# ComputationalRobotics/XM-code

Measured on AMD Instinct MI355X. Metric: BM iters/sec (tCG Hessian-vector iterations per second; ms_per_step = wall-clock-to-KKT of one staircase solve), higher is better.
Workload: dtype f64

## Files before the change

xm-code_amd/csrc/xm_common.h:

```cpp
#pragma once

#include <hip/hip_runtime.h>

#include <cstdint>
#include <cstdio>
#include <stdexcept>
#include <string>
#include <vector>

namespace xm {

struct Error : std::runtime_error {
    int code;
    Error(int c, const std::string &m) : std::runtime_error(m), code(c) {}
};

#define XM_HIP_CHECK(expr)                                                                            \
    do {                                                                                              \
        hipError_t _e = (expr);                                                                       \
        if (_e != hipSuccess)                                                                         \
            throw ::xm::Error(-3, std::string("HIP error: ") + hipGetErrorString(_e) + " at " +       \
                                      __FILE__ + ":" + std::to_string(__LINE__) + " (" #expr ")");    \
    } while (0)

// ... 76 lines not shown
    double *ksum;
    unsigned int *kcount;
    int nt_cam0;
    int rev;
    struct Cand { const double *R, *s; double *G, *egs, *S0, *rgR, *rgs, *partials; } cand;
};

enum Epilogue { EPI_PLAIN = 0, EPI_GRAD = 1, EPI_HESS = 2, EPI_CERT = 3, EPI_AUTO = 4 };
__host__ __device__ inline CamArgs cand_args(const CamArgs &a) {
    CamArgs b = a;
    b.R = a.cand.R; b.s = a.cand.s; b.G = a.cand.G; b.egs = a.cand.egs; b.S0 = a.cand.S0; b.rgR = a.cand.rgR; b.rgs = a.cand.rgs;
    b.partials = a.cand.partials;
    return b;
}

constexpr int kMaxPeers = 8;
struct PeerXchg {
    int world = 0, rank = 0;
    double *buf[kMaxPeers] = {};
    unsigned long long *flag[kMaxPeers] = {};
    unsigned long long *ticket = nullptr;
    unsigned long long *err = nullptr;
    long long spin_ticks = 0;
    unsigned long long epoch_base = 0;
    int mute = 0;
    int lite = 0;
};

struct PointPtrs { double *G, *egs, *S0, *rgR, *rgs; };
struct OuterStepArgs {
    int nloc, cam0;
    const TcgScal *scal_cur;
    TcgScal *scal_next;
    const OuterScal *os_cur;
    OuterScal *os_next;
    const double *parts;
    double *partsB_out;
    int nA, nB;
    const double *HpR, *Hps;
    double *R, *s;
    double *Rc, *sc;
    double *pR;
    const double *ps_cur;
    double *ps_next;
    double *vR, *vs, *HvR, *Hvs, *rR;
    const double *rs_cur;
    double *rs_next;
    double *Wloc, *Wpad;
    PointPtrs cur, cand;
    const double *partsA;
    double *partsM;
    int nM;
    double delta_bar, gradtol;
    int max_outer;
    double *trace;
    int trace_cap;
    const int *stop_req;
    unsigned long long *hprog;
    unsigned int run;
    int slot, grp;
};
void launch_outer_step(int o, int polar, const OuterStepArgs &A, int grid, hipStream_t st);

void launch_qw_dense(int o, int epi, const double *Q, int64_t ld, const double *W, double alpha, const CamArgs &a,
                     hipStream_t st);
void launch_qw_bsr3(int o, int epi, const int64_t *rowptr, const int32_t *colidx, const double *blocks, const double *W,
                    double alpha, const CamArgs &a, hipStream_t st, int64_t nb = 0, const int4 *rowinfo = nullptr);
int64_t sell_resident_bytes(int64_t stream, int64_t other);
void bsr_build_rowinfo(const int64_t *rowptr_host, int nloc, std::vector<int4> &out);
int qw_grid(int nloc);
void launch_qw_dense_split(int o, int epi, const double *Q, int64_t ld, const double *W, double alpha, const CamArgs &a, hipStream_t st);
int qw_dense_tile_cols();
int qw_dense_split_k(int nloc, int64_t ld);
int bsr_grid(int nloc);
size_t sym_prow_count(int nloc, int64_t ld, int o);
size_t sym_pcol_count(int nloc, int64_t ld, int o);
void qw_bench_nt(int nt);
void symv_bench_k(int k, int kf);
int symv_trace_slots();
void launch_qw_sym_traced(int o, const double *Q, int64_t ld, const double *W, const CamArgs &a, double *Prow, double *Pcol, unsigned long long *trace,
                          int grid[2], hipStream_t st);
void symv_plan_get(int nloc, int64_t ld, int out[4]);
void launch_qw_sym(int o, int epi, const double *Q, int64_t ld, const double *W, double alpha, const CamArgs &a, double *Prow,
                   double *Pcol, hipStream_t st, int rev = 0);
void launch_asym(const double *Q, int64_t ld, int64_t m, double *out, int grid, hipStream_t st);
void launch_dense_to_f32(const double *src, float *dst, int64_t rows, int64_t ld, unsigned int *bad, hipStream_t st);
void launch_qw_dense_f32(int o, int epi, const float *Qf, const double *Qd, int64_t ld, const double *W, double alpha, const CamArgs &a, hipStream_t st);
void launch_qw_sym_f32(int o, int epi, const float *Qf, const double *Qd, int64_t ld, const double *W, double alpha, const CamArgs &a, double *Prow,
                       double *Pcol, hipStream_t st, int rev = 0);

void launch_symhash(const double *Q, int64_t ld, int64_t row0, int64_t nrows, int64_t m, unsigned long long *out, int grid, hipStream_t st);

void launch_transpose_pad(const double *src_colmajor, int64_t lds, int64_t rows, int64_t cols, double *dst, int64_t ldd,
                          hipStream_t st);
void launch_dense_from_bsr(const int64_t *rowptr, const int32_t *colidx, const double *blocks, int64_t nloc, int64_t cam0,
                           double *dst, int64_t ldd, hipStream_t st);

int flat_grid(int64_t elems);
void launch_scale_rows(int o, int nloc, const double *R, const double *s, double *Wloc, hipStream_t st);
void launch_tcg_init(int o, int nloc, const double *rgR, const double *rgs, const double *R, const double *s, double *rR,
                     double *rs, double *pR, double *ps, double *vR, double *vs, double *HvR, double *Hvs, double *Wloc,
                     TcgScal *scal0, double rr, double delta, unsigned long long *hstat, hipStream_t st, double *Wpad = nullptr, int seq = 0,
                     const SpecCtl *spec = nullptr);
void launch_cg_step(int o, int nloc, const TcgScal *scal_cur, TcgScal *scal_next, const double *parts, int nA_loc, int nB_loc, int world,
                    const double *HpR, const double *Hps, const double *R, const double *s, double *pR,
                    const double *ps_cur, double *ps_next, double *vR, double *vs, double *HvR, double *Hvs, double *rR, const double *rs_cur,
                    double *rs_next, double *Wloc, double *partsB_out, unsigned long long *hstat, int b_off, int64_t mat, double *Afull,
                    double *Wfull, int grouping, const struct PeerXchg &xchg, hipStream_t st, double *Wpad = nullptr);
struct OuterArgs { double loss, delta, delta_bar, gradtol; int shrink_count, last_iter; };
void launch_outer_finalize(const double *partsA, int nA_loc, int world, const double *partsM, int nM, const TcgScal *scal, double *hres,
                           unsigned long long seq, int grouping, hipStream_t st, const OuterArgs *oa = nullptr, SpecCtl *spec_out = nullptr);
void launch_retract(int o, int nloc, int cam0, const double *R, const double *s, const double *D, const double *ds, double t,
                    double *Rout, double *sout, double *Wloc, hipStream_t st, int polar = 0);
int retract_grid(int nloc);
void launch_retract_model(int o, int nloc, int cam0, const double *R, const double *s, const double *vR, const double *vs, double *Rout, double *sout,
                          double *Wloc, double *Wpad, const double *HvR, const double *Hvs, const double *rgR, const double *rgs, double *parts,
                          hipStream_t st, int polar);
void launch_cert_prepare(int o, int nloc, int cam0, double lam, const double *QsR, const double *R, const double *s,
                         double *Lam, double *dz, double *parts, hipStream_t st);
void launch_recover_gram(int64_t n, int r, const double *R, const double *s, double *parts, int grid, hipStream_t st);
void launch_recover_project(int64_t n, int r, const double *R, const double *s, const double *V, double *rot, double *scale, int *negcount,
                            hipStream_t st, int variant = 0);
void launch_negate(double *x, int64_t len, hipStream_t st);
int dots_multi_segments(int64_t len);
void launch_dots_multi(const double *V, int64_t ldv, int m, const double *w, int64_t len, double *c, double *scratch, hipStream_t st);
void launch_sub_vc(double *w, const double *V, int64_t ldv, const double *c, int m, int64_t len, hipStream_t st);
void launch_scale_copy(double *dst, const double *src, double a, int64_t len, hipStream_t st);
void launch_copy_words(void *dst, const void *src, size_t bytes, hipStream_t st);
void launch_lz_alpha(const double *c1j, const double *c2j, double *alpha_j, hipStream_t st);
void launch_dots_multi_parts(const double *V, int64_t ldv, int m, const double *w, int64_t len, double *scratch, hipStream_t st);
bool lz_fused_ok(int m);
void launch_sub_vc_fin(double *w, const double *V, int64_t ldv, const double *parts, int m, int64_t len, double *c_out, const double *c_prev,
                       double *alpha_j, hipStream_t st);
void launch_lz_next_fin(double *dst, const double *w, const double *parts, double *beta_j, int64_t len, hipStream_t st);
void launch_lz_next(double *dst, const double *w, const double *ww, double *beta_j, int64_t len, hipStream_t st);
void launch_gemv_n(double *y, const double *V, int64_t ldv, const double *c, int m, int64_t len, hipStream_t st);


void launch_edge_locate(int64_t ne, const int32_t *ei, const int32_t *ej, int cam0, int nloc, const int64_t *rowptr, const int32_t *colidx,
                        int64_t *pos_ij, int64_t *pos_ji, int64_t *pos_d, hipStream_t st);
void launch_edge_write(bool dense, int64_t ne, const int32_t *ei, const int32_t *ej, const double *M, const double *w, int cam0, int nloc,
                       const int64_t *inc_ptr, const int32_t *inc_edge, const int64_t *pos_ij, const int64_t *pos_ji, const int64_t *pos_d,
                       double *blocks, double *Q, int64_t ld, hipStream_t st);
void launch_edge_residual(int64_t ne, const int32_t *ei, const int32_t *ej, const double *M, const double *Y, int o, int OP, double *res,
                          hipStream_t st);

void launch_xm2_error(int64_t n, const double *w, const double *res, double *err, hipStream_t st);
void launch_radix_hist(int64_t n, const double *x, int shift, unsigned long long prefix, unsigned int *hist, hipStream_t st);
void launch_xm2_filter(int64_t n, const double *err, const double *w, double thr, double *wout, unsigned int *removed, hipStream_t st);

#define XM_DISPATCH_O(o, CALL)                                                         \
    switch (o) {                                                                       \
        case 1: { constexpr int O_ = 1; CALL; } break;                                 \
        case 3: { constexpr int O_ = 3; CALL; } break;                                 \
        case 4: { constexpr int O_ = 4; CALL; } break;                                 \
        case 5: { constexpr int O_ = 5; CALL; } break;                                 \
        case 6: { constexpr int O_ = 6; CALL; } break;                                 \
        case 7: { constexpr int O_ = 7; CALL; } break;                                 \
        case 8: { constexpr int O_ = 8; CALL; } break;                                 \
        case 9: { constexpr int O_ = 9; CALL; } break;                                 \
        case 10: { constexpr int O_ = 10; CALL; } break;                               \
        default: throw Error(-2, "rank o must be 1 or 3..10, got " + std::to_string(o)); \
    }

inline void check_launch(const char *what) {
    hipError_t e = hipGetLastError();
    if (e != hipSuccess) throw Error(-3, std::string("kernel launch failed (") + what + "): " + hipGetErrorString(e));
}

}
```

xm-code_amd/csrc/xm_kernels.hip:

```cpp
#include <algorithm>
#include <cmath>
#include <cstdlib>
#include <cstring>
#include <type_traits>

#include "xm_common.h"
#include "xm_device.h"

namespace xm {

__device__ __forceinline__ double2 nt_load16(const double2 *p) {
    typedef double d2v __attribute__((ext_vector_type(2)));
    const d2v v = __builtin_nontemporal_load(reinterpret_cast<const d2v *>(p));
    return make_double2(v.x, v.y);
}

template <int O, int EPI, int NSUB, bool SPLIT = false>
__global__ __launch_bounds__(256) void qw_dense_kernel(const double *__restrict__ Q, int64_t ld,
                                                        const double *__restrict__ W, double alpha, CamArgs a) {
    constexpr int OP = pitch_of(O);
    int role = EPI;
    constexpr int TILE = NSUB * 128;
    constexpr int TILE2 = TILE * OP / 2;
    constexpr int NST = (TILE2 + 255) / 256;
// ... 743 lines not shown
                for (int k = 0; k < O; ++k) acc[r][k] += q[3 * r] * w[0][k] + q[3 * r + 1] * w[1][k] + q[3 * r + 2] * w[2][k];
        }
        if (VAR >= 1) {
            __builtin_amdgcn_fence(__ATOMIC_ACQ_REL, "wavefront");
            __builtin_amdgcn_wave_barrier();
        }
    }
    EpiOps eops;
    BSR_TS(5);
    epi_prefetch<O, EPI>(eops, active ? cam : 0, gl, active, a, (EPI == EPI_AUTO) ? role : (int)EPI);
    qw_finish<O, EPI, 16, kBsrRows>(cam, gl, slot, active, acc, alpha, a, eops, red, (EPI == EPI_AUTO) ? role : (int)EPI);
    BSR_TS(6);
}
#ifdef XM_BSR_TRACE
extern "C" void xm_bsr_trace_set(unsigned long long *p) { (void)hipMemcpyToSymbol(HIP_SYMBOL(g_bsr_trace), &p, sizeof(p)); }
#endif

__global__ __launch_bounds__(256) void transpose_pad_kernel(const double *__restrict__ src, int64_t lds, int64_t rows,
                                                             int64_t cols, double *__restrict__ dst, int64_t ldd) {
    __shared__ double tile[32][33];
    const int tx = threadIdx.x & 31, ty = threadIdx.x >> 5;
    const int64_t r0 = (int64_t)blockIdx.y * 32, c0 = (int64_t)blockIdx.x * 32;
#pragma unroll
    for (int j = 0; j < 32; j += 8) {
        const int64_t r = r0 + tx, c = c0 + ty + j;
        tile[ty + j][tx] = (r < rows && c < cols) ? src[r + c * lds] : 0.0;
    }
    __syncthreads();
#pragma unroll
    for (int j = 0; j < 32; j += 8) {
        const int64_t r = r0 + ty + j, c = c0 + tx;
        if (r < rows && c < ldd) dst[r * ldd + c] = (c < cols) ? tile[tx][ty + j] : 0.0;
    }
}

__global__ void dense_from_bsr_kernel(const int64_t *__restrict__ rowptr, const int32_t *__restrict__ colidx,
                                      const double *__restrict__ blocks, int64_t nloc, int64_t cam0, double *dst, int64_t ldd) {
    const int64_t cam = blockIdx.x;
    if (cam >= nloc) return;
    for (int64_t b = rowptr[cam0 + cam] + threadIdx.x / 9; b < rowptr[cam0 + cam + 1]; b += blockDim.x / 9) {
        const int e = threadIdx.x % 9;
        if (threadIdx.x / 9 < (int)(blockDim.x / 9))
            dst[(cam * 3 + e / 3) * ldd + (int64_t)colidx[b] * 3 + e % 3] = blocks[b * 9 + e];
    }
}

#pragma clang fp contract(off)
__device__ __forceinline__ unsigned long long pack_stat(int seq, int iter, int status) {
    return ((unsigned long long)(unsigned)seq << 32) | ((unsigned long long)((unsigned)iter & 0xffffffu) << 8) | (unsigned long long)(unsigned)(status & 0xff);
}
__device__ __forceinline__ void publish_host(unsigned long long *hstat, unsigned long long v) {
    if (hstat) __hip_atomic_store(hstat, v, __ATOMIC_RELAXED, __HIP_MEMORY_SCOPE_SYSTEM);
}

struct StepDecision {
    int mode;
    double step;
};
__device__ __forceinline__ StepDecision tcg_decide(const TcgScal &sc, double pHp) {
    StepDecision d;
    const double alpha = sc.rr / pHp;
    if (sc.rr < 1e-15) { d.mode = 5; d.step = 0.0; return d; }
    const bool neg = alpha <= 0.0;
    if (neg || sc.vv + 2.0 * alpha * sc.vp + alpha * alpha * sc.pp > sc.delta * sc.delta) {
        const double sq = sqrt(sc.vp * sc.vp + sc.pp * (sc.delta * sc.delta - sc.vv));
        d.mode = neg ? 1 : 2;
        d.step = (-sc.vp + sq) / sc.pp;
        return d;
    }
    d.mode = 0; d.step = alpha;
    return d;
}

template <int O>
__global__ __launch_bounds__(256) void scale_rows_kernel(int nloc, const double *__restrict__ R, const double *__restrict__ s,
                                                          double *__restrict__ Wloc) {
    constexpr int OP = pitch_of(O);
    const int64_t total = (int64_t)nloc * 3 * OP;
    for (int64_t i = (int64_t)blockIdx.x * 256 + threadIdx.x; i < total; i += (int64_t)gridDim.x * 256)
        Wloc[i] = R[i] * s[i / (3 * OP)];
}

template <int O>
__global__ __launch_bounds__(256) void tcg_init_kernel(int nloc, const double *__restrict__ rgR, const double *__restrict__ rgs,
                                                        const double *__restrict__ R, const double *__restrict__ s,
                                                        double *rR, double *rs, double *pR, double *ps, double *vR, double *vs,
                                                        double *HvR, double *Hvs, double *Wloc, TcgScal *scal0, double rr,
                                                        double delta, unsigned long long *hstat, double *Wpad, int seq, const SpecCtl *spec) {
    constexpr int OP = pitch_of(O);
    const int64_t total = (int64_t)nloc * 3 * OP;
    if (spec != nullptr) {
        if (!spec->go) {
            if (blockIdx.x == 0 && threadIdx.x == 0) { TcgScal sc = *scal0; sc.status = 9; sc.seq = seq; *scal0 = sc; }
            return;
        }
        rr = spec->rr; delta = spec->delta;
    }
    for (int64_t i = (int64_t)blockIdx.x * 256 + threadIdx.x; i < total; i += (int64_t)gridDim.x * 256) {
        const int cam = (int)(i / (3 * OP));
        const double g = rgR[i], gs = rgs[cam];
        rR[i] = g; pR[i] = -g; vR[i] = 0.0; HvR[i] = 0.0;
        const double wv = s[cam] * (-g) + (-gs) * R[i];
        if (Wloc) Wloc[i] = wv;
        if (Wpad) Wpad[(size_t)cam * 16 + (i - (int64_t)cam * (3 * OP))] = wv;
        if (i % (3 * OP) == 0) { rs[cam] = gs; ps[cam] = -gs; vs[cam] = 0.0; Hvs[cam] = 0.0; }
    }
    if (blockIdx.x == 0 && threadIdx.x == 0) {
        TcgScal sc = {};
        sc.rr = rr; sc.vv = 0.0; sc.vp = 0.0; sc.pp = rr; sc.delta = delta; sc.gradnorm = sqrt(rr); sc.last_step = 0.0; sc.model = 0.0;
        sc.status = 0; sc.iter = 0; sc.seq = seq;
        *scal0 = sc;
        publish_host(hstat, pack_stat(seq, 0, 0));
    }
}

template <int O>
__global__ __launch_bounds__(256) void cg_step_kernel(int nloc, const TcgScal *__restrict__ scal_cur, TcgScal *scal_next,
                                                       const double *__restrict__ parts, int nA_loc, int nB_loc, int world,
                                                       const double *__restrict__ HpR,
                                                       const double *__restrict__ Hps, const double *__restrict__ R,
                                                       const double *__restrict__ s, double *pR, const double *__restrict__ ps_cur,
                                                       double *ps_next, double *vR, double *vs, double *HvR, double *Hvs, double *rR,
                                                       const double *__restrict__ rs_cur, double *rs_next, double *Wloc,
                                                       double *partsB_out, unsigned long long *hstat, int b_off, int64_t mat,
                                                       double *Afull, double *Wfull, int grp, PeerXchg x, double *Wpad) {
    constexpr int OP = pitch_of(O);
    __shared__ double sh[4];
    __shared__ double sh16[16];
    __shared__ int sh_flag;
    const int64_t total = (int64_t)nloc * 3 * OP;
    const int64_t stride = (int64_t)gridDim.x * 256;
    int64_t i = (int64_t)blockIdx.x * 256 + threadIdx.x;
    const bool in0 = i < total;
    const int camf = (int)(i / (3 * OP));
    const bool own0 = in0 && (i % (3 * OP) == 0);
    double hp = 0, pv = 0, vv0 = 0, hv = 0, rv = 0, Rv = 0, hs = 0, psv = 0, rsv = 0, sv = 1, vsv = 0, hvs = 0;
    const bool keep_hv = HvR != nullptr;
    if (in0) { hp = HpR[i]; pv = pR[i]; vv0 = vR[i]; if (keep_hv) hv = HvR[i]; rv = rR[i]; Rv = R[i]; hs = Hps[camf]; psv = ps_cur[camf]; rsv = rs_cur[camf]; sv = s[camf]; }
    if (own0) { vsv = vs[camf]; if (keep_hv) hvs = Hvs[camf]; }
    const bool can_pre = x.world <= 1;
    PartialsPre pre;
    if (can_pre) sum_partials_prefetch(parts + b_off, parts + b_off + nA_loc, parts + b_off + 2 * nA_loc, nA_loc, parts + b_off + 3 * nA_loc, nB_loc, pre, grp);
    const TcgScal sc0 = *scal_cur;
    const bool lead = (blockIdx.x == 0 && threadIdx.x == 0);
    if (sc0.status != 0) {
        if (lead) *scal_next = sc0;
        return;
    }
    if (x.world > 1) {
        const int par = sc0.iter & 1;
        const size_t chunk_d = (size_t)b_off + 3 * (size_t)nA_loc + nB_loc;
        const size_t off = ((size_t)par * x.world + x.rank) * chunk_d;
        const unsigned long long epoch = x.epoch_base + (unsigned long long)sc0.iter + 1ull;
        const double *src = x.buf[x.rank] + off;
        if (x.lite) {
            for (int p = 0; p < x.world; ++p) {
                if (p == x.rank) continue;
                double *dst = x.buf[p] + off;
                for (size_t j = (size_t)blockIdx.x * 256 + threadIdx.x; j < chunk_d; j += (size_t)stride)
                    __hip_atomic_store(dst + j, src[j], __ATOMIC_RELAXED, __HIP_MEMORY_SCOPE_SYSTEM);
            }
            asm volatile("s_waitcnt vmcnt(0)" ::: "memory");
            __syncthreads();
            if (threadIdx.x == 0) {
                const unsigned long long t = __hip_atomic_fetch_add(x.ticket + par, 1ull, __ATOMIC_RELAXED, __HIP_MEMORY_SCOPE_AGENT);
                sh_flag = (t + 1 == gridDim.x);
                if (sh_flag) __hip_atomic_store(x.ticket + par, 0ull, __ATOMIC_RELAXED, __HIP_MEMORY_SCOPE_AGENT);
            }
            __syncthreads();
            if (sh_flag && !x.mute && threadIdx.x < x.world && (int)threadIdx.x != x.rank)
                __hip_atomic_store(x.flag[threadIdx.x] + par * kMaxPeers + x.rank, epoch, __ATOMIC_RELAXED, __HIP_MEMORY_SCOPE_SYSTEM);
        } else {
            for (int p = 0; p < x.world; ++p) {
                if (p == x.rank) continue;
                double *dst = x.buf[p] + off;
                for (size_t j = (size_t)blockIdx.x * 256 + threadIdx.x; j < chunk_d; j += (size_t)stride) dst[j] = src[j];
            }
            __threadfence_system();
            asm volatile("s_waitcnt vmcnt(0)" ::: "memory");
            __syncthreads();
            if (threadIdx.x == 0) {
                const unsigned long long t = __hip_atomic_fetch_add(x.ticket + par, 1ull, __ATOMIC_ACQ_REL, __HIP_MEMORY_SCOPE_AGENT);
                sh_flag = (t + 1 == gridDim.x);
                if (sh_flag) __hip_atomic_store(x.ticket + par, 0ull, __ATOMIC_RELAXED, __HIP_MEMORY_SCOPE_AGENT);
            }
            __syncthreads();
            if (sh_flag && !x.mute && threadIdx.x < x.world && (int)threadIdx.x != x.rank) {
                __threadfence_system();
                asm volatile("s_waitcnt vmcnt(0)" ::: "memory");
// ... 64 lines not shown
            const double rsn = rsv + step * hs;
            rR[i] = rn;
            acc += rn * rn;
            if (newdir) {
                const double pn = beta * pv - rn;
                const double psn = beta * psv - rsn;
                pR[i] = pn;
                if (!Afull) {
                    const double wv = sv * pn + psn * Rv;
                    if (Wloc) Wloc[i] = wv;
                    if (Wpad) Wpad[(size_t)camf * 16 + (i - (int64_t)camf * (3 * OP))] = wv;
                }
                if (own0) ps_next[camf] = psn;
            }
            if (own0) { rs_next[camf] = rsn; const double q = rsn / sv; acc += q * q; }
        }
        if (own0) { vs[camf] = vsv + step * psv; if (keep_hv) Hvs[camf] = hvs + step * hs; }
    }
    for (i += stride; i < total; i += stride) {
        const int cam = (int)(i / (3 * OP));
        const bool own = (i % (3 * OP) == 0);
        const double hpi = HpR[i], pi = pR[i], hsi = Hps[cam], psi = ps_cur[cam];
        vR[i] += step * pi;
        if (keep_hv) HvR[i] += step * hpi;
        if (cg) {
            const double rn = rR[i] + step * hpi;
            const double rsn = rs_cur[cam] + step * hsi;
            rR[i] = rn;
            acc += rn * rn;
            if (newdir) {
                const double pn = beta * pi - rn;
                const double psn = beta * psi - rsn;
                pR[i] = pn;
                if (!Afull) {
                    const double wv = s[cam] * pn + psn * R[i];
                    if (Wloc) Wloc[i] = wv;
                    if (Wpad) Wpad[(size_t)cam * 16 + (i - (int64_t)cam * (3 * OP))] = wv;
                }
                if (own) ps_next[cam] = psn;
            }
            if (own) { rs_next[cam] = rsn; const double q = rsn / s[cam]; acc += q * q; }
        }
        if (own) { vs[cam] += step * psi; if (keep_hv) Hvs[cam] += step * hsi; }
    }
    if (Afull && newdir) {
        const int64_t full = mat * world;
        const bool first = (sc0.iter == 0);
        for (int64_t j = (int64_t)blockIdx.x * 256 + threadIdx.x; j < full; j += stride) {
            const int64_t r = j / mat;
            const double b = parts[(size_t)r * chunk + (size_t)(j - r * mat)];
            const double w = Wfull[j];
            const double an = (first ? -w : Afull[j]) + step * b;
            Afull[j] = an;
            Wfull[j] = beta * w - an;
        }
    }
    if (cg) {
        const double tot = block_sum256(acc, sh);
        if (threadIdx.x == 0) partsB_out[blockIdx.x] = tot;
    }
    if (lead) {
        TcgScal nx = sc;
        nx.last_step = step;
        if (!keep_hv) nx.model = sc.model - step * sc.rr + 0.5 * step * step * pHp;
        if (!cg) {
            nx.status = d.mode;
        } else {
            nx.rr = rr_est;
            nx.vv = sc.vv + 2.0 * step * sc.vp + step * step * sc.pp;
            nx.vp = beta * (sc.vp + step * sc.pp);
            nx.pp = beta * beta * sc.pp + rr_est;
            if (conv) {
                nx.status = 3;
            } else {
                nx.iter = sc.iter + 1;
                nx.status = (nx.iter >= kMaxInner) ? 6 : 0;
            }
        }
        *scal_next = nx;
        publish_host(hstat, pack_stat(nx.seq, nx.iter, nx.status));
    }
}

__global__ __launch_bounds__(256) void outer_finalize_kernel(const double *__restrict__ partsA, int nA_loc, int world,
                                                              const double *__restrict__ partsM, int nM,
                                                              const TcgScal *__restrict__ scal, double *hres, unsigned long long seq, int grp,
                                                              OuterArgs oa, SpecCtl *spec_out) {
    __shared__ double sh[4];
    double f = 0.0, rr = 0.0;
    for (int r = 0; r < world; ++r) {
        f += sum_partials256(partsA + (size_t)r * 2 * nA_loc, nA_loc, sh, grp);
        rr += sum_partials256(partsA + (size_t)r * 2 * nA_loc + nA_loc, nA_loc, sh, grp);
    }
    const double m_vec = (nM > 0) ? sum_partials256(partsM, nM, sh, grp) : 0.0;
    if (threadIdx.x == 0) {
        const TcgScal sc = *scal;
        const double m = (nM > 0) ? m_vec : sc.model;
        __hip_atomic_store(hres + 0, f, __ATOMIC_RELAXED, __HIP_MEMORY_SCOPE_SYSTEM);
        __hip_atomic_store(hres + 1, rr, __ATOMIC_RELAXED, __HIP_MEMORY_SCOPE_SYSTEM);
        __hip_atomic_store(hres + 2, m, __ATOMIC_RELAXED, __HIP_MEMORY_SCOPE_SYSTEM);
        __hip_atomic_store(hres + 3, (double)sc.status, __ATOMIC_RELAXED, __HIP_MEMORY_SCOPE_SYSTEM);
        __hip_atomic_store(hres + 4, (double)sc.iter, __ATOMIC_RELAXED, __HIP_MEMORY_SCOPE_SYSTEM);
        if (spec_out != nullptr) {
            const int endreason = (sc.status == 0) ? 6 : sc.status;
            double delta = oa.delta;
            int shrink = oa.shrink_count;
            bool go = (m < 0.0) && endreason != 7;
            if (go) {
                const double rou = (f - oa.loss) / m;
                if (rou < 0.25) { delta *= 0.25; shrink++; }
                else if (rou > 0.75 && endreason <= 2) { delta = fmin(delta * 2, oa.delta_bar); shrink = 0; }
                else shrink = 0;
                bool stop_delta = false;
                if (shrink > 3) { delta *= 1e-3; shrink = 0; if (delta < 1e-20) stop_delta = true; }
                const bool reject = (f > oa.loss || rou < 0.1);
                go = !stop_delta && !reject && endreason != 5 && !(sqrt(rr) < oa.gradtol) && !oa.last_iter;
            }
            SpecCtl sp;
            sp.go = go ? 1 : 0; sp.pad_ = 0; sp.rr = rr; sp.delta = delta;
            *spec_out = sp;
            __hip_atomic_store(hres + 6, go ? 1.0 : 0.0, __ATOMIC_RELAXED, __HIP_MEMORY_SCOPE_SYSTEM);
            __hip_atomic_store(hres + 7, delta, __ATOMIC_RELAXED, __HIP_MEMORY_SCOPE_SYSTEM);
        }
        __atomic_thread_fence(__ATOMIC_SEQ_CST);
        asm volatile("s_waitcnt vmcnt(0)" ::: "memory");
        __hip_atomic_store(reinterpret_cast<unsigned long long *>(hres + 5), seq, __ATOMIC_RELEASE, __HIP_MEMORY_SCOPE_SYSTEM);
    }
}

__device__ __forceinline__ double det3(const double (&M)[3][3]);
template <int O>
__device__ __forceinline__ void polar_rows(double (&X)[3][O]) {
    for (int it = 0; it < 40; ++it) {
        double G[3][3];
#pragma unroll
        for (int a = 0; a < 3; ++a)
#pragma unroll
            for (int b = a; b < 3; ++b) {
                double tt = 0.0;
#pragma unroll
                for (int k = 0; k < O; ++k) tt += X[a][k] * X[b][k];
                G[a][b] = tt; G[b][a] = tt;
            }
        const double d = det3(G);
        if (!(d > 0.0)) return;
        double C[3][3];
        C[0][0] = G[1][1] * G[2][2] - G[1][2] * G[2][1]; C[0][1] = G[0][2] * G[2][1] - G[0][1] * G[2][2]; C[0][2] = G[0][1] * G[1][2] - G[0][2] * G[1][1];
        C[1][1] = G[0][0] * G[2][2] - G[0][2] * G[2][0]; C[1][2] = G[0][2] * G[1][0] - G[0][0] * G[1][2]; C[2][2] = G[0][0] * G[1][1] - G[0][1] * G[1][0];
        C[1][0] = C[0][1]; C[2][0] = C[0][2]; C[2][1] = C[1][2];
        double Y[3][O], nx = 0.0, ny = 0.0;
#pragma unroll
        for (int a = 0; a < 3; ++a)
#pragma unroll
            for (int k = 0; k < O; ++k) {
                const double y = (C[a][0] * X[0][k] + C[a][1] * X[1][k] + C[a][2] * X[2][k]) / d;
                Y[a][k] = y; nx += X[a][k] * X[a][k]; ny += y * y;
            }
        const double g = sqrt(sqrt(ny / nx));
        double delta = 0.0;
#pragma unroll
        for (int a = 0; a < 3; ++a)
#pragma unroll
            for (int k = 0; k < O; ++k) {
                const double z = 0.5 * (g * X[a][k] + Y[a][k] / g);
                delta += (z - X[a][k]) * (z - X[a][k]);
                X[a][k] = z;
            }
        if (delta < 1e-31) return;
    }
}

template <int O, int POLAR>
__device__ __forceinline__ void retract_rows(double (&q)[3][O]) {
    if constexpr (POLAR) {
        polar_rows<O>(q);
    } else {
#pragma unroll
        for (int i = 0; i < 3; ++i) {
            double qq = 0.0;
#pragma unroll
            for (int k = 0; k < O; ++k) qq += q[i][k] * q[i][k];
            qq = sqrt(qq);
#pragma unroll
            for (int k = 0; k < O; ++k) q[i][k] /= qq;
#pragma unroll
            for (int j = i + 1; j < 3; ++j) {
                double uu = 0.0;
#pragma unroll
                for (int k = 0; k < O; ++k) uu += q[i][k] * q[j][k];
#pragma unroll
                for (int k = 0; k < O; ++k) q[j][k] -= uu * q[i][k];
            }
        }
    }
}

struct ModelArgs { const double *HvR, *Hvs, *rgR, *rgs; double *parts; };
template <int O, int POLAR, bool MV = false>
__global__ __launch_bounds__(256) void retract_kernel(int nloc, int cam0, const double *__restrict__ R, const double *__restrict__ s,
                                                       const double *__restrict__ D, const double *__restrict__ ds, double t,
                                                       double *Rout, double *sout, double *Wloc, double *Wpad, ModelArgs mv) {
    constexpr int OP = pitch_of(O);
    __shared__ double sh_mv[4];
    const int cam = blockIdx.x * 256 + threadIdx.x;
    const bool live = cam < nloc;
    if constexpr (!MV) {
        if (!live) return;
    }
    const size_t base = (size_t)(live ? cam : 0) * 3 * OP;
    double q[3][O];
// ... 952 lines not shown
    }
}
void launch_qw_dense(int o, int epi, const double *Q, int64_t ld, const double *W, double alpha, const CamArgs &a, hipStream_t st) {
    if (a.nloc <= 0) return;
    if (a.ks > 1 && a.ksum && a.kcount) {
        XM_DISPATCH_O(o, (qw_dense_ks_o<O_>(epi, Q, ld, W, alpha, a, st)));
        check_launch("qw_dense_ks");
        return;
    }
    if (epi == EPI_CERT) {
        if (o != 1) throw Error(-2, "certificate operator needs o == 1");
        CamArgs ac = a;
        ac.nt_cam0 = qw_nt_cam0(a.nloc, ld);
        hipLaunchKernelGGL((qw_dense_kernel<1, EPI_CERT, 2>), dim3(qw_grid(a.nloc)), dim3(256), 0, st, Q, ld, W, alpha, ac);
    } else {
        XM_DISPATCH_O(o, (qw_dense_epi<O_, kQwNsub>(epi, Q, ld, W, alpha, a, st)));
    }
    check_launch("qw_dense");
}

static int64_t symv_live_groups(int64_t nsteps, int64_t nstrips, int64_t k) {
    int64_t live = 0;
    for (int64_t s = 0; s < nstrips; ++s) live += (std::min<int64_t>(nsteps, (s * kSvStrip + kSvStrip + 5) / 6) + 4 * k - 1) / (4 * k);
    return live;
}
int symv_k(int nloc, int64_t ld) {
    const int64_t nsteps = (nloc + 1) / 2, nstrips = (ld + kSvStrip - 1) / kSvStrip;
    int64_t total = 0;
    for (int64_t s = 0; s < nstrips; ++s) total += std::min<int64_t>(nsteps, (s * kSvStrip + kSvStrip + 5) / 6);
    int64_t k = (int64_t)(std::sqrt((double)total) / 18.0 + 0.5);
    k = std::min<int64_t>(64, std::max<int64_t>(2, k));
    if (symv_live_groups(nsteps, nstrips, k) <= 1100) {
        int64_t ks = 4;
        while (symv_live_groups(nsteps, nstrips, ks) > 504) ++ks;
        k = ks;
    }
    return (int)k;
}
size_t sym_prow_count(int nloc, int64_t ld, int o) { return (size_t)((ld + kSvStrip - 1) / kSvStrip) * 6 * (size_t)((nloc + 1) / 2) * o; }
static int g_symv_k = 0, g_symv_kf = 0;
void symv_bench_k(int k, int kf) { g_symv_k = k; g_symv_kf = kf; }
struct SymvPlan { int K, Kf, ysplit, nchunks, gx, gy; };
static SymvPlan symv_plan(int nloc, int64_t ld) {
    SymvPlan p;
    p.K = g_symv_k > 0 ? g_symv_k : symv_k(nloc, ld);
    const int nsteps = (nloc + 1) / 2, nstrips = (int)((ld + kSvStrip - 1) / kSvStrip);
    p.gy = (nstrips + 1) / 2;
    if (g_symv_k > 0 && g_symv_kf > 0) {
        p.Kf = std::min(g_symv_kf, p.K);
        p.ysplit = (int)(0.75 * p.gy);
    } else if (p.K >= 8 && symv_live_groups(nsteps, nstrips, p.K) > 1100) {
        p.Kf = p.K / 4;
        p.ysplit = (int)(0.75 * p.gy);
    } else {
        p.Kf = p.K; p.ysplit = p.gy;
    }
    auto groups = [&](int s, int k) { return (int)((std::min<int64_t>(nsteps, ((int64_t)s * kSvStrip + kSvStrip + 5) / 6) + 4 * k - 1) / (4 * k)); };
    p.gx = 1;
    for (int y = 0; y < p.gy; ++y) {
        const int k = (y >= p.ysplit) ? p.Kf : p.K, sb = nstrips - 1 - y;
        p.gx = std::max(p.gx, groups(y, k) + (sb != y ? groups(sb, k) : 0));
    }
    p.nchunks = (nsteps + 4 * p.Kf - 1) / (4 * p.Kf);
    return p;
}
void symv_plan_get(int nloc, int64_t ld, int out[4]) {
    const SymvPlan p = symv_plan(nloc, ld);
    out[0] = p.K; out[1] = p.Kf; out[2] = p.ysplit; out[3] = p.nchunks;
}
size_t sym_pcol_count(int nloc, int64_t ld, int o) { return (size_t)symv_plan(nloc, ld).nchunks * (size_t)ld * o; }

static int symv_nt_step0(int nloc, int64_t ld) {
    const double m = 3.0 * nloc;
    const double tri = 8.0 * m * (m + 6.0) / 2.0;
    const int64_t res = qw_resident_bytes((size_t)tri);
    const int nsteps = (nloc + 1) / 2;
    if ((double)res >= tri) return nsteps + 1;
    const double disc = m * m - 2.0 * (double)res / 8.0;
    const double r = m - std::sqrt(std::max(0.0, disc));
    return (int)std::min<double>(nsteps + 1, std::max(0.0, r / 6.0));
}
template <int O>
static void qw_symv_epi(int epi, const double *Q, int64_t ld, const double *W, double alpha, const CamArgs &a, double *Prow, double *Pcol,
                        hipStream_t st, int rev, unsigned long long *trace = nullptr) {
    const SymvPlan pl = symv_plan(a.nloc, ld);
    const int nstrips = (int)((ld + kSvStrip - 1) / kSvStrip);
    const TcgScal *sc = (epi == EPI_HESS || epi == EPI_AUTO) ? a.scal : (const TcgScal *)nullptr;
    const int by_phase = (epi == EPI_AUTO) ? 1 : 0;
    const int ys = pl.ysplit, rK = 4 * pl.K, rKf = 4 * pl.Kf, rys = ys;
    const dim3 gs(pl.gx, pl.gy);
    const int nt0 = symv_nt_step0(a.nloc, ld);
    if (trace) {
        if constexpr (O == 3 || O == 4) hipLaunchKernelGGL((qw_symv_kernel<O, true>), gs, dim3(256), 0, st, Q, ld, W, a.nloc, pl.K, pl.Kf, ys, nt0, sc, Prow, Pcol, trace, rev, by_phase);
    } else hipLaunchKernelGGL((qw_symv_kernel<O>), gs, dim3(256), 0, st, Q, ld, W, a.nloc, pl.K, pl.Kf, ys, nt0, sc, Prow, Pcol, trace, rev, by_phase);
    const dim3 g(qw_grid(a.nloc)), b(256);
    switch (epi) {
        case EPI_PLAIN: hipLaunchKernelGGL((symv_reduce_kernel<O, EPI_PLAIN>), g, b, 0, st, Prow, Pcol, ld, nstrips, rK, rKf, rys, alpha, a); break;
        case EPI_GRAD: hipLaunchKernelGGL((symv_reduce_kernel<O, EPI_GRAD>), g, b, 0, st, Prow, Pcol, ld, nstrips, rK, rKf, rys, alpha, a); break;
        case EPI_HESS: hipLaunchKernelGGL((symv_reduce_kernel<O, EPI_HESS>), g, b, 0, st, Prow, Pcol, ld, nstrips, rK, rKf, rys, alpha, a); break;
        case EPI_AUTO:
            if constexpr (O >= 3) { hipLaunchKernelGGL((symv_reduce_kernel<O, EPI_AUTO>), g, b, 0, st, Prow, Pcol, ld, nstrips, rK, rKf, rys, alpha, a); break; }
            throw Error(-2, "bad epilogue");
        case EPI_CERT:
            if constexpr (O == 1) { hipLaunchKernelGGL((symv_reduce_kernel<1, EPI_CERT>), g, b, 0, st, Prow, Pcol, ld, nstrips, rK, rKf, rys, alpha, a); break; }
            throw Error(-2, "certificate operator needs o == 1");
        default: throw Error(-2, "bad epilogue");
    }
}
int symv_trace_slots() { return kSvTraceSlots; }
void launch_qw_sym_traced(int o, const double *Q, int64_t ld, const double *W, const CamArgs &a, double *Prow, double *Pcol, unsigned long long *trace,
                          int grid[2], hipStream_t st) {
    const SymvPlan pl = symv_plan(a.nloc, ld);
    grid[0] = pl.gx; grid[1] = pl.gy;
    if (trace == nullptr) return;
    if (o == 3) qw_symv_epi<3>(EPI_PLAIN, Q, ld, W, 1.0, a, Prow, Pcol, st, 0, trace);
    else if (o == 4) qw_symv_epi<4>(EPI_PLAIN, Q, ld, W, 1.0, a, Prow, Pcol, st, 0, trace);
    else throw Error(-2, "traced symmetric product: o = 3 or 4");
    check_launch("qw_symv traced");
}

void launch_qw_sym(int o, int epi, const double *Q, int64_t ld, const double *W, double alpha, const CamArgs &a, double *Prow,
                   double *Pcol, hipStream_t st, int rev) {
    if (a.nloc <= 0) return;
    switch (o) {
        case 1: qw_symv_epi<1>(epi, Q, ld, W, alpha, a, Prow, Pcol, st, rev & 1); break;
        case 3: qw_symv_epi<3>(epi, Q, ld, W, alpha, a, Prow, Pcol, st, rev & 1); break;
        case 4: qw_symv_epi<4>(epi, Q, ld, W, alpha, a, Prow, Pcol, st, rev & 1); break;
        case 5: qw_symv_epi<5>(epi, Q, ld, W, alpha, a, Prow, Pcol, st, rev & 1); break;
        default: throw Error(-2, "symmetric product is instantiated for o = 1, 3..5");
    }
    check_launch("qw_symv");
}
__global__ __launch_bounds__(256) void symhash_kernel(const double *__restrict__ Q, int64_t ld, int64_t row0, int64_t nrows, int64_t m,
                                                       unsigned long long *out) {
    __shared__ unsigned long long sh[2][4];
    unsigned long long acc = 0ull, bad = 0ull;
    const int64_t total = nrows * m;
    for (int64_t e = (int64_t)blockIdx.x * 256 + threadIdx.x; e < total; e += (int64_t)gridDim.x * 256) {
        const int64_t lr = e / m, c = e - lr * m, r = row0 + lr;
        if (r >= m || r == c) continue;
        const double v = Q[lr * ld + c];
        if (v != v) bad = 1ull;
        unsigned long long b = (v == 0.0) ? 0ull : (unsigned long long)__double_as_longlong(v);
        unsigned long long z = (unsigned long long)((r < c) ? r : c) * 0x9E3779B97F4A7C15ull + (unsigned long long)((r < c) ? c : r);
        z = (z ^ (z >> 30)) * 0xBF58476D1CE4E5B9ull; z = (z ^ (z >> 27)) * 0x94D049BB133111EBull; z ^= z >> 31;
        const unsigned long long t = (z | 1ull) * b;
        acc += (r < c) ? t : (0ull - t);
    }
    for (int off = 32; off > 0; off >>= 1) { acc += __shfl_xor(acc, off, 64); bad |= __shfl_xor(bad, off, 64); }
    if ((threadIdx.x & 63) == 0) { sh[0][threadIdx.x >> 6] = acc; sh[1][threadIdx.x >> 6] = bad; }
    __syncthreads();
    if (threadIdx.x == 0) {
        out[2 * blockIdx.x] = sh[0][0] + sh[0][1] + sh[0][2] + sh[0][3];
        out[2 * blockIdx.x + 1] = sh[1][0] | sh[1][1] | sh[1][2] | sh[1][3];
    }
}
void launch_symhash(const double *Q, int64_t ld, int64_t row0, int64_t nrows, int64_t m, unsigned long long *out, int grid, hipStream_t st) {
    hipLaunchKernelGGL(symhash_kernel, dim3(grid), dim3(256), 0, st, Q, ld, row0, nrows, m, out);
    check_launch("symhash");
}
void launch_asym(const double *Q, int64_t ld, int64_t m, double *out, int grid, hipStream_t st) {
    hipLaunchKernelGGL(asym_kernel, dim3(grid), dim3(256), 0, st, Q, ld, m, out);
    check_launch("asym");
}

template <int O, int VAR>
static void qw_bsr3_epi(int epi, const int64_t *rp, const int32_t *ci, const double *bl, const double *W, const int4 *ri, double alpha,
                        const CamArgs &a, hipStream_t st) {
    const dim3 g((a.nloc + kBsrRows - 1) / kBsrRows), b(256);
    switch (epi) {
        case EPI_PLAIN: hipLaunchKernelGGL((qw_bsr3_kernel<O, EPI_PLAIN, VAR>), g, b, 0, st, rp, ci, bl, W, ri, alpha, a); break;
        case EPI_GRAD: hipLaunchKernelGGL((qw_bsr3_kernel<O, EPI_GRAD, VAR>), g, b, 0, st, rp, ci, bl, W, ri, alpha, a); break;
        case EPI_HESS: hipLaunchKernelGGL((qw_bsr3_kernel<O, EPI_HESS, VAR>), g, b, 0, st, rp, ci, bl, W, ri, alpha, a); break;
        case EPI_AUTO:
            if constexpr (O >= 3) { hipLaunchKernelGGL((qw_bsr3_kernel<O, EPI_AUTO, VAR>), g, b, 0, st, rp, ci, bl, W, ri, alpha, a); break; }
            throw Error(-2, "bad epilogue");
        default: throw Error(-2, "bad epilogue");
    }
}
static int bsr_nt_cam0(int nloc, int64_t nb) {
    const size_t bytes = (size_t)std::max<int64_t>(nb, 0) * 76;
    return qw_resident_bytes(bytes) >= (int64_t)bytes ? nloc : 0;
}
void bsr_build_rowinfo(const int64_t *rowptr_host, int nloc, std::vector<int4> &out) {
    out.resize((size_t)std::max(nloc, 0));
    for (int c0 = 0; c0 < nloc; c0 += kBsrRows) {
        const int m = std::min(kBsrRows, nloc - c0);
        int order[kBsrRows];
        for (int j = 0; j < m; ++j) order[j] = c0 + j;
        std::stable_sort(order, order + m, [&](int x, int y) {
            return (rowptr_host[x + 1] - rowptr_host[x] + 15) / 16 > (rowptr_host[y + 1] - rowptr_host[y] + 15) / 16;
        });
        for (int j = 0; j < m; ++j) {
            const int i = order[j];
            const int64_t b0 = rowptr_host[i], len = rowptr_host[i + 1] - b0;
            if (len >= ((int64_t)1 << 31)) throw Error(-2, "block-CSR row with 2^31 or more blocks");
            out[(size_t)c0 + j] = make_int4((int)(unsigned)(b0 & 0xffffffffll), (int)(unsigned)((unsigned long long)b0 >> 32), (int)len, i);
        }
    }
}
void launch_qw_bsr3(int o, int epi, const int64_t *rp, const int32_t *ci, const double *bl, const double *W, double alpha,
                    const CamArgs &a0, hipStream_t st, int64_t nb, const int4 *ri) {
    if (a0.nloc <= 0) return;
    CamArgs a = a0;
    a.nt_cam0 = bsr_nt_cam0(a.nloc, nb);
    if (epi == EPI_CERT) {
        if (o != 1) throw Error(-2, "certificate operator needs o == 1");
        hipLaunchKernelGGL((qw_bsr3_kernel<1, EPI_CERT, 0>), dim3((a.nloc + kBsrRows - 1) / kBsrRows), dim3(256), 0, st, rp, ci, bl, W, ri, alpha, a);
    } else {
        switch (o) {
            case 3: qw_bsr3_epi<3, 2>(epi, rp, ci, bl, W, ri, alpha, a, st); break;
            case 4: qw_bsr3_epi<4, 2>(epi, rp, ci, bl, W, ri, alpha, a, st); break;
            case 5: qw_bsr3_epi<5, 2>(epi, rp, ci, bl, W, ri, alpha, a, st); break;
            case 6: qw_bsr3_epi<6, 2>(epi, rp, ci, bl, W, ri, alpha, a, st); break;
            case 1: qw_bsr3_epi<1, 1>(epi, rp, ci, bl, W, ri, alpha, a, st); break;
            case 7: qw_bsr3_epi<7, 1>(epi, rp, ci, bl, W, ri, alpha, a, st); break;
            case 8: qw_bsr3_epi<8, 1>(epi, rp, ci, bl, W, ri, alpha, a, st); break;
            case 9: qw_bsr3_epi<9, 1>(epi, rp, ci, bl, W, ri, alpha, a, st); break;
            case 10: qw_bsr3_epi<10, 1>(epi, rp, ci, bl, W, ri, alpha, a, st); break;
            default: throw Error(-2, "rank o must be 1 or 3..10, got " + std::to_string(o));
        }
    }
    check_launch("qw_bsr3");
}

void launch_transpose_pad(const double *src, int64_t lds, int64_t rows, int64_t cols, double *dst, int64_t ldd, hipStream_t st) {
    const dim3 g((unsigned)((ldd + 31) / 32), (unsigned)((rows + 31) / 32));
    hipLaunchKernelGGL(transpose_pad_kernel, g, dim3(256), 0, st, src, lds, rows, cols, dst, ldd);
    check_launch("transpose_pad");
}
void launch_dense_from_bsr(const int64_t *rp, const int32_t *ci, const double *bl, int64_t nloc, int64_t cam0, double *dst,
                           int64_t ldd, hipStream_t st) {
    hipLaunchKernelGGL(dense_from_bsr_kernel, dim3((unsigned)nloc), dim3(252), 0, st, rp, ci, bl, nloc, cam0, dst, ldd);
    check_launch("dense_from_bsr");
}

void launch_scale_rows(int o, int nloc, const double *R, const double *s, double *Wloc, hipStream_t st) {
    XM_DISPATCH_O(o, hipLaunchKernelGGL((scale_rows_kernel<O_>), dim3(flat_grid((int64_t)nloc * 3 * pitch_of(O_))), dim3(256), 0, st,
                                        nloc, R, s, Wloc));
    check_launch("scale_rows");
}
void launch_tcg_init(int o, int nloc, const double *rgR, const double *rgs, const double *R, const double *s, double *rR, double *rs,
                     double *pR, double *ps, double *vR, double *vs, double *HvR, double *Hvs, double *Wloc, TcgScal *scal0,
                     double rr, double delta, unsigned long long *hstat, hipStream_t st, double *Wpad, int seq, const SpecCtl *spec) {
    XM_DISPATCH_O(o, hipLaunchKernelGGL((tcg_init_kernel<O_>), dim3(flat_grid((int64_t)nloc * 3 * pitch_of(O_))), dim3(256), 0, st,
                                        nloc, rgR, rgs, R, s, rR, rs, pR, ps, vR, vs, HvR, Hvs, Wloc, scal0, rr, delta, hstat, Wpad, seq, spec));
    check_launch("tcg_init");
}
void launch_cg_step(int o, int nloc, const TcgScal *scal_cur, TcgScal *scal_next, const double *parts, int nA_loc, int nB_loc, int world,
                    const double *HpR, const double *Hps, const double *R, const double *s, double *pR,
                    const double *ps_cur, double *ps_next, double *vR, double *vs, double *HvR, double *Hvs, double *rR, const double *rs_cur,
                    double *rs_next, double *Wloc, double *partsB_out, unsigned long long *hstat, int b_off, int64_t mat, double *Afull,
                    double *Wfull, int grouping, const PeerXchg &xchg, hipStream_t st, double *Wpad) {
    XM_DISPATCH_O(o, hipLaunchKernelGGL((cg_step_kernel<O_>), dim3(nB_loc), dim3(256), 0, st, nloc,
                                        scal_cur, scal_next, parts, nA_loc, nB_loc, world, HpR, Hps, R, s, pR, ps_cur, ps_next, vR,
                                        vs, HvR, Hvs, rR, rs_cur, rs_next, Wloc, partsB_out, hstat, b_off, mat, Afull, Wfull, grouping, xchg, Wpad));
    check_launch("cg_step");
}
void launch_outer_finalize(const double *partsA, int nA_loc, int world, const double *partsM, int nM, const TcgScal *scal, double *hres,
                           unsigned long long seq, int grouping, hipStream_t st, const OuterArgs *oa, SpecCtl *spec_out) {
    OuterArgs z;
    std::memset(&z, 0, sizeof(z));
    hipLaunchKernelGGL(outer_finalize_kernel, dim3(1), dim3(256), 0, st, partsA, nA_loc, world, partsM, nM, scal, hres, seq, grouping, oa ? *oa : z,
                       (oa != nullptr) ? spec_out : (SpecCtl *)nullptr);
    check_launch("outer_finalize");
}
void launch_outer_step(int o, int polar, const OuterStepArgs &A, int grid, hipStream_t st) {
    switch (o) {
#define XM_OS_CASE(OO) case OO: if (polar) hipLaunchKernelGGL((outer_step_kernel<OO, 1>), dim3(grid), dim3(256), 0, st, A); \
                                else hipLaunchKernelGGL((outer_step_kernel<OO, 0>), dim3(grid), dim3(256), 0, st, A); break;
        XM_OS_CASE(3) XM_OS_CASE(4) XM_OS_CASE(5) XM_OS_CASE(6) XM_OS_CASE(7) XM_OS_CASE(8) XM_OS_CASE(9) XM_OS_CASE(10)
#undef XM_OS_CASE
        default: throw Error(-2, "device-driven outer iteration: rank o must be 3..10, got " + std::to_string(o));
    }
    check_launch("outer_step");
}
int retract_grid(int nloc) { return (nloc + 255) / 256; }
void launch_retract_model(int o, int nloc, int cam0, const double *R, const double *s, const double *vR, const double *vs, double *Rout, double *sout,
                          double *Wloc, double *Wpad, const double *HvR, const double *Hvs, const double *rgR, const double *rgs, double *parts,
                          hipStream_t st, int polar) {
    const ModelArgs mv = {HvR, Hvs, rgR, rgs, parts};
    const dim3 g(retract_grid(nloc)), b(256);
    if (HvR == nullptr) {
        if (polar) { XM_DISPATCH_O(o, hipLaunchKernelGGL((retract_kernel<O_, 1, false>), g, b, 0, st, nloc, cam0, R, s, vR, vs, 1.0, Rout, sout, Wloc, Wpad, mv)); }
        else { XM_DISPATCH_O(o, hipLaunchKernelGGL((retract_kernel<O_, 0, false>), g, b, 0, st, nloc, cam0, R, s, vR, vs, 1.0, Rout, sout, Wloc, Wpad, mv)); }
        check_launch("retract");
        return;
    }
    if (polar) { XM_DISPATCH_O(o, hipLaunchKernelGGL((retract_kernel<O_, 1, true>), g, b, 0, st, nloc, cam0, R, s, vR, vs, 1.0, Rout, sout, Wloc, Wpad, mv)); }
    else { XM_DISPATCH_O(o, hipLaunchKernelGGL((retract_kernel<O_, 0, true>), g, b, 0, st, nloc, cam0, R, s, vR, vs, 1.0, Rout, sout, Wloc, Wpad, mv)); }
    check_launch("retract_model");
}
void launch_retract(int o, int nloc, int cam0, const double *R, const double *s, const double *D, const double *ds, double t,
                    double *Rout, double *sout, double *Wloc, hipStream_t st, int polar) {
    const ModelArgs mv = {nullptr, nullptr, nullptr, nullptr, nullptr};
    if (polar == 2) {
        XM_DISPATCH_O(o, hipLaunchKernelGGL((retract_quad_kernel<O_>), dim3((nloc + 63) / 64), dim3(256), 0, st, nloc, cam0, R, s, D, ds, t,
                                            Rout, sout, Wloc));
    } else if (polar) {
        XM_DISPATCH_O(o, hipLaunchKernelGGL((retract_kernel<O_, 1>), dim3((nloc + 255) / 256), dim3(256), 0, st, nloc, cam0, R, s, D, ds, t,
                                            Rout, sout, Wloc, (double *)nullptr, mv));
    } else {
        XM_DISPATCH_O(o, hipLaunchKernelGGL((retract_kernel<O_, 0>), dim3((nloc + 255) / 256), dim3(256), 0, st, nloc, cam0, R, s, D, ds, t,
                                            Rout, sout, Wloc, (double *)nullptr, mv));
    }
    check_launch("retract");
}
void launch_cert_prepare(int o, int nloc, int cam0, double lam, const double *QsR, const double *R, const double *s, double *Lam,
                         double *dz, double *parts, hipStream_t st) {
    XM_DISPATCH_O(o, hipLaunchKernelGGL((cert_prepare_kernel<O_>), dim3((nloc + 255) / 256), dim3(256), 0, st, nloc, cam0, lam, QsR, R,
                                        s, Lam, dz, parts));
    check_launch("cert_prepare");
}
void launch_recover_gram(int64_t n, int r, const double *R, const double *s, double *parts, int grid, hipStream_t st) {
    hipLaunchKernelGGL(recover_gram_kernel, dim3(grid), dim3(256), 0, st, n, r, R, s, parts);
    check_launch("recover_gram");
}
void launch_recover_project(int64_t n, int r, const double *R, const double *s, const double *V, double *rot, double *scale, int *negcount,
                            hipStream_t st, int variant) {
    if (variant == 1) hipLaunchKernelGGL(recover_project_wave_kernel, dim3((unsigned)((n + 3) / 4)), dim3(256), 0, st, n, r, R, s, V, rot, scale, negcount);
    else hipLaunchKernelGGL(recover_project_kernel, dim3((unsigned)((n + 255) / 256)), dim3(256), 0, st, n, r, R, s, V, rot, scale, negcount);
    check_launch("recover_project");
}
void launch_negate(double *x, int64_t len, hipStream_t st) {
    hipLaunchKernelGGL(negate_kernel, dim3(flat_grid(len)), dim3(256), 0, st, x, len);
    check_launch("negate");
}
int dots_multi_segments(int64_t len) { return (int)std::min<int64_t>(64, std::max<int64_t>(1, len / 4096)); }
void launch_dots_multi(const double *V, int64_t ldv, int m, const double *w, int64_t len, double *c, double *scratch, hipStream_t st) {
    if (m <= 0) return;
    const int nseg = dots_multi_segments(len);
    if (nseg <= 1 || !scratch) {
        hipLaunchKernelGGL(dots_multi_kernel, dim3(m), dim3(256), 0, st, V, ldv, w, len, c);
    } else {
        const int64_t seg = ((len + nseg - 1) / nseg + 255) / 256 * 256;
        hipLaunchKernelGGL(dots_multi_seg_kernel, dim3(m, nseg), dim3(256), 0, st, V, ldv, w, len, seg, scratch);
        hipLaunchKernelGGL(dots_multi_fin_kernel, dim3((m + 255) / 256), dim3(256), 0, st, scratch, m, nseg, c);
    }
    check_launch("dots_multi");
}
void launch_dots_multi_parts(const double *V, int64_t ldv, int m, const double *w, int64_t len, double *scratch, hipStream_t st) {
    if (m <= 0) return;
    const int nseg = dots_multi_segments(len);
    const int64_t seg = ((len + nseg - 1) / nseg + 255) / 256 * 256;
    hipLaunchKernelGGL(dots_multi_seg_kernel, dim3(m, nseg), dim3(256), 0, st, V, ldv, w, len, seg, scratch);
    check_launch("dots_multi_parts");
}
bool lz_fused_ok(int m) { return m <= kLzMaxCols; }
// ... 354 lines not shown
                run(at(i), qA, wA);
                load_q(at(i + 2), qA, wA);
                run(at(i + 1), qB, wB);
                i += 2;
            }
            if (i + 1 < cnt) {
                load_q(at(i + 1), qB, wB);
                run(at(i), qA, wA);
                run(at(i + 1), qB, wB);
            } else {
                run(at(i), qA, wA);
            }
        }
        return true;
    };
    bool alive;
    const bool nt = jb >= nt_step0;
    if constexpr (AUTO) {
        const int ph = scal->phase;
        if (ph >= PH_STOP) return;
        if (ph == PH_CAND) alive = nt ? sweep(Qd, std::true_type{}) : sweep(Qd, std::false_type{});
        else alive = nt ? sweep(Qf, std::true_type{}) : sweep(Qf, std::false_type{});
    } else {
        alive = nt ? sweep(Qf, std::true_type{}) : sweep(Qf, std::false_type{});
    }
    if (!alive) return;
#pragma unroll
    for (int h = 0; h < 2; ++h)
#pragma unroll
        for (int e = 0; e < 2; ++e)
#pragma unroll
            for (int k = 0; k < O; ++k) L[((h * 2 + e) * O + k) * 64 + lane] = ca[h][e][k];
    __syncthreads();
    if (wave < 2 && lane_ok) {
        double *pc = Pcol + ((size_t)sc * (size_t)ld + (size_t)(cA + 2 * wave)) * O;
#pragma unroll
        for (int e = 0; e < 2; ++e)
#pragma unroll
            for (int k = 0; k < O; ++k) {
                const int idx = ((wave * 2 + e) * O + k) * 64 + lane;
                pc[e * O + k] = ((lds[0][idx] + lds[1][idx]) + lds[2][idx]) + lds[3][idx];
            }
    }
}

void launch_dense_to_f32(const double *src, float *dst, int64_t rows, int64_t ld, unsigned int *bad, hipStream_t st) {
    if (ld % 4 != 0) throw Error(-2, "fp32 copy: leading dimension must be a multiple of 4");
    const size_t n4 = (size_t)rows * (size_t)ld / 4;
    XM_HIP_CHECK(hipMemsetAsync(bad, 0, sizeof(unsigned int), st));
    if (n4 == 0) return;
    const int grid = (int)std::min<size_t>(4096, (n4 + 255) / 256);
    hipLaunchKernelGGL(dense_to_f32_kernel, dim3(grid), dim3(256), 0, st, src, dst, n4, bad);
    check_launch("dense_to_f32");
}

template <int O>
static void qw_dense_f32_epi(int epi, const float *Qf, const double *Qd, int64_t ld, const double *W, double alpha, const CamArgs &a0, hipStream_t st) {
    const dim3 g(qw_grid(a0.nloc)), b(256);
    CamArgs a = a0;
    {
        const size_t row3 = (size_t)3 * (size_t)ld * sizeof(float);
        a.nt_cam0 = (int)std::min<int64_t>(a.nloc, qw_resident_bytes((size_t)a.nloc * row3) / (int64_t)row3);
    }
    switch (epi) {
        case EPI_PLAIN: hipLaunchKernelGGL((qw_dense_f32_kernel<O, EPI_PLAIN>), g, b, 0, st, Qf, Qd, ld, W, alpha, a); break;
        case EPI_HESS: hipLaunchKernelGGL((qw_dense_f32_kernel<O, EPI_HESS>), g, b, 0, st, Qf, Qd, ld, W, alpha, a); break;
        case EPI_AUTO:
            if constexpr (O >= 3) {
                if (!Qd) throw Error(-2, "fp32 product in the device-driven role needs the f64 matrix too");
                hipLaunchKernelGGL((qw_dense_f32_kernel<O, EPI_AUTO>), g, b, 0, st, Qf, Qd, ld, W, alpha, a);
                break;
            }
            throw Error(-2, "bad epilogue");
        default: throw Error(-2, "fp32 dense product: plain, Hessian or device-driven epilogue only");
    }
}
void launch_qw_dense_f32(int o, int epi, const float *Qf, const double *Qd, int64_t ld, const double *W, double alpha, const CamArgs &a, hipStream_t st) {
    if (a.nloc <= 0) return;
    XM_DISPATCH_O(o, (qw_dense_f32_epi<O_>(epi, Qf, Qd, ld, W, alpha, a, st)));
    check_launch("qw_dense_f32");
}
template <int O>
static void qw_symv_f32_epi(int epi, const float *Qf, const double *Qd, int64_t ld, const double *W, double alpha, const CamArgs &a, double *Prow,
                            double *Pcol, hipStream_t st, int rev) {
    const SymvPlan pl = symv_plan(a.nloc, ld);
    const int nstrips = (int)((ld + kSvStrip - 1) / kSvStrip);
    const int rK = 4 * pl.K, rKf = 4 * pl.Kf, ys = pl.ysplit;
    const dim3 gs(pl.gx, pl.gy), g(qw_grid(a.nloc)), b(256);
    int nt0;
    {
        const double m = 3.0 * a.nloc, tri = 4.0 * m * (m + 6.0) / 2.0;
        const int64_t res = qw_resident_bytes((size_t)tri);
        const int nsteps = (a.nloc + 1) / 2;
        if ((double)res >= tri) nt0 = nsteps + 1;
        else {
            const double r = m - std::sqrt(std::max(0.0, m * m - 2.0 * (double)res / 4.0));
            nt0 = (int)std::min<double>(nsteps + 1, std::max(0.0, r / 6.0));
        }
    }
    switch (epi) {
        case EPI_PLAIN:
            hipLaunchKernelGGL((qw_symv_f32_kernel<O, false>), gs, b, 0, st, Qf, Qd, ld, W, a.nloc, pl.K, pl.Kf, ys, nt0, (const TcgScal *)nullptr, Prow, Pcol, rev);
            hipLaunchKernelGGL((symv_reduce_kernel<O, EPI_PLAIN>), g, b, 0, st, Prow, Pcol, ld, nstrips, rK, rKf, ys, alpha, a);
            break;
        case EPI_HESS:
            hipLaunchKernelGGL((qw_symv_f32_kernel<O, false>), gs, b, 0, st, Qf, Qd, ld, W, a.nloc, pl.K, pl.Kf, ys, nt0, a.scal, Prow, Pcol, rev);
            hipLaunchKernelGGL((symv_reduce_kernel<O, EPI_HESS>), g, b, 0, st, Prow, Pcol, ld, nstrips, rK, rKf, ys, alpha, a);
            break;
        case EPI_AUTO:
            if constexpr (O >= 3) {
                if (!Qd) throw Error(-2, "fp32 product in the device-driven role needs the f64 matrix too");
                const int nt64 = symv_nt_step0(a.nloc, ld);
                hipLaunchKernelGGL((qw_symv_f32_kernel<O, true>), gs, b, 0, st, Qf, Qd, ld, W, a.nloc, pl.K, pl.Kf, ys, std::min(nt0, nt64), a.scal, Prow, Pcol, rev);
                hipLaunchKernelGGL((symv_reduce_kernel<O, EPI_AUTO>), g, b, 0, st, Prow, Pcol, ld, nstrips, rK, rKf, ys, alpha, a);
                break;
            }
            throw Error(-2, "bad epilogue");
        default: throw Error(-2, "fp32 symmetric product: plain, Hessian or device-driven epilogue only");
    }
}
void launch_qw_sym_f32(int o, int epi, const float *Qf, const double *Qd, int64_t ld, const double *W, double alpha, const CamArgs &a, double *Prow,
                       double *Pcol, hipStream_t st, int rev) {
    if (a.nloc <= 0) return;
    switch (o) {
        case 3: qw_symv_f32_epi<3>(epi, Qf, Qd, ld, W, alpha, a, Prow, Pcol, st, rev & 1); break;
        case 4: qw_symv_f32_epi<4>(epi, Qf, Qd, ld, W, alpha, a, Prow, Pcol, st, rev & 1); break;
        case 5: qw_symv_f32_epi<5>(epi, Qf, Qd, ld, W, alpha, a, Prow, Pcol, st, rev & 1); break;
        default: throw Error(-2, "fp32 symmetric product is instantiated for o = 3..5");
    }
    check_launch("qw_symv_f32");
}

}
```

xm-code_amd/csrc/xm_sell.h:

```cpp
#pragma once

#include <cstdint>
#include <vector>

#include "xm_solver.h"

namespace xm {

struct SellHost {
    int64_t nloc = 0, ncols = 0;
    int S = 1, lmax = 0;
    bool slice_order = true;
    int64_t nvrows = 0, nslices = 0, nsteps = 0, nparts = 0, nstore = 0;
    std::vector<int64_t> slice_off;
    std::vector<int32_t> slab_start;
    std::vector<uint8_t> kind;
    std::vector<int64_t> src;
    std::vector<int32_t> pslot;
    std::vector<int32_t> ridx;
    std::vector<int64_t> pptr;
    int64_t lines_native72 = 0, lines_native120 = 0, lines_padded = 0;
    std::vector<int64_t> diag_src;
};

void sell_build_host(const int64_t *rowptr, const int32_t *colidx, int64_t nloc, int64_t ncols, int S, int lmax, SellHost &out,
                     int64_t diag_row0 = -1);

enum { SELL_CODEC_FULL = 0, SELL_CODEC_QUAT = 1 };
constexpr int64_t kSellMinBlocks = 2200000;

struct SellArgs {
    const int64_t *slice_off;
    const int32_t *slab_start;
    const int32_t *cols;
    const double *blk;
    const double *diag;
    int64_t row0;
    const int32_t *pslot;
    const int64_t *pptr;
    const int32_t *ridx;
    int S;
    int wstride;
    int coalesced_store;
    int64_t nt_off;
};

class SellMatrix {
public:
    int64_t ncols() const { return ncols_; }
    bool padded_pays(int o) const { return o >= 3 && 3 * pitch_of(o) <= 16 && lines_padded_ * 11 < (3 * pitch_of(o) <= 9 ? lines72_ : lines120_) * 10; }
    SellMatrix(const int64_t *rowptr, const int32_t *colidx, const double *blocks, int64_t nloc, int64_t ncols, int S, int lmax,
               hipStream_t st, int codec = SELL_CODEC_FULL, int64_t row0 = 0);
    int codec() const { return codec_; }
    int64_t stream_bytes() const;
    int64_t nt_off(int o, int64_t nloc) const;
    SellArgs args() const;
    void refill(const int32_t *d_colidx, const double *d_blocks, hipStream_t st);
    double *parts(int o);
    int wstride(int o) const;
    int reduce_gw(int o) const;
    int reduce_grid(int o, int nloc) const;
    int grid() const { return grid_; }
    int64_t nloc() const { return nloc_; }
    int64_t nparts() const { return nparts_; }
    int64_t nsteps() const { return nsteps_; }
    int S() const { return S_; }

private:
    int64_t nloc_ = 0, nparts_ = 0, nsteps_ = 0, nslices_ = 0;
    int S_ = 1, grid_ = 0;
    int64_t ncols_ = 0, max_list_ = 0;
    int64_t lines72_ = 0, lines120_ = 0, lines_padded_ = 0;
    bool coalesced_ = false;
    DevBuf<int64_t> slice_off_, pptr_;
    DevBuf<int32_t> slab_start_, cols_, pslot_, ridx_;
    DevBuf<double> blk_, parts_;
    DevBuf<int64_t> src_;
    DevBuf<uint8_t> kind_;
    int64_t b0_ = 0;
    int parts_o_ = 0;
    int codec_ = SELL_CODEC_FULL;
    int64_t row0_ = 0;
    DevBuf<double> diag_;
    DevBuf<int64_t> diag_src_;
};

void check_viewgraph_blocks(const int64_t *rowptr, const int32_t *colidx, const double *blocks, int64_t nloc, int64_t row0);
void launch_qw_sell(int o, int epi, SellMatrix &m, const double *W, double alpha, const CamArgs &a, int gm, hipStream_t st,
                    const double *Wpad16 = nullptr);
bool sell_supports(int o);
void sell_quat_roundtrip(const double block[9], double quat[4], double rebuilt[9]);

}
```

xm-code_amd/csrc/xm_sell.hip:

```cpp
#include "xm_sell.h"

#include <algorithm>
#include <cstdlib>
#include <cstring>
#include <numeric>
#include <type_traits>

#include "xm_device.h"
#include "xm_sell_codec.h"

namespace xm {

void sell_build_host(const int64_t *rowptr, const int32_t *colidx, int64_t nloc, int64_t ncols, int S, int lmax, SellHost &out,
                     int64_t diag_row0) {
    if (!(S == 1 || S == 2 || S == 4 || S == 8)) throw Error(XM_ERR_ARG, "SELL: slabs must be 1, 2, 4 or 8");
    if (lmax < 2) throw Error(XM_ERR_ARG, "SELL: lmax must be >= 2");
    if (nloc < 0 || ncols < 1 || !rowptr) throw Error(XM_ERR_ARG, "SELL: bad sizes");
    out = SellHost();
    out.nloc = nloc; out.ncols = ncols; out.S = S; out.lmax = lmax;
    const int64_t b0 = rowptr[0], nb = rowptr[nloc] - b0;
    if (nb < 0) throw Error(XM_ERR_ARG, "BSR3: rowptr is not monotone");
    if (nb > 0 && !colidx) throw Error(XM_ERR_ARG, "BSR3: colidx missing");
    std::vector<int64_t> order;
    order.reserve((size_t)nb);
// ... 516 lines not shown
}
template <int GM>
__global__ __launch_bounds__(256) __attribute__((amdgpu_waves_per_eu(4, 4))) void qw_sell_kernel_q_occ4(SellArgs m, const double *__restrict__ W,
                                                                                                      const TcgScal *__restrict__ scal,
                                                                                                      double *__restrict__ parts) {
    qw_sell_entry<3, GM, 0, SELL_CODEC_QUAT>(m, W, scal, parts);
}

int SellMatrix::reduce_gw(int o) const { return (o <= 4 && max_list_ <= 32) ? 4 : 16; }
int SellMatrix::reduce_grid(int o, int nloc) const { const int per = 256 / reduce_gw(o); return (nloc + per - 1) / per; }

template <int O, int EPI, int GW>
__global__ __launch_bounds__(256) void sell_reduce_kernel(const int64_t *__restrict__ pptr, const int32_t *__restrict__ ridx, const double *__restrict__ parts,
                                                           double alpha, CamArgs a, const double *__restrict__ diag, const double *__restrict__ W,
                                                           int64_t row0, int wstride) {
    constexpr int NSLOT = 256 / GW;
    __shared__ double red[NSLOT][3];
    const int gl = threadIdx.x & (GW - 1), slot = threadIdx.x / GW;
    const int cam = blockIdx.x * NSLOT + slot;
    const bool active = cam < a.nloc;
    EpiOps eops;
    epi_prefetch<O, EPI>(eops, active ? cam : 0, gl, active, a);
    const int64_t p0 = active ? pptr[cam] : 0, p1 = active ? pptr[cam + 1] : 0;
    if (EPI == EPI_HESS) {
        if (a.scal->status != 0) return;
    }
    double acc[3][O];
#pragma unroll
    for (int r = 0; r < 3; ++r)
#pragma unroll
        for (int k = 0; k < O; ++k) acc[r][k] = 0.0;
    if (active) {
        for (int64_t p = p0 + gl; p < p1; p += GW) {
            const double *v = parts + (size_t)ridx[p] * 3 * O;
#pragma unroll
            for (int r = 0; r < 3; ++r)
#pragma unroll
                for (int k = 0; k < O; ++k) acc[r][k] += v[r * O + k];
        }
        if (diag != nullptr && !(EPI == EPI_HESS && a.Bout == nullptr) && gl == GW - 1) {
            constexpr int OPW = pitch_of(O);
            const double d = diag[cam];
            const double *w = W + (size_t)(row0 + cam) * wstride;
#pragma unroll
            for (int r = 0; r < 3; ++r)
#pragma unroll
                for (int k = 0; k < O; ++k) acc[r][k] = fma(d, w[r * OPW + k], acc[r][k]);
        }
    }
    if constexpr (EPI == EPI_HESS) {
        if (diag != nullptr && a.Bout == nullptr) {
            Col3 h;
            h.v[0] = h.v[1] = h.v[2] = 0.0;
#pragma unroll
            for (int r = 0; r < 3; ++r)
#pragma unroll
                for (int k = 0; k < O; ++k) {
                    const double t = group_sum<GW>(acc[r][k]);
                    if (gl == k) h.v[r] = t;
                }
            if (active && gl < O) {
                const double d = diag[cam];
#pragma unroll
                for (int r = 0; r < 3; ++r) h.v[r] = alpha * fma(d, eops.s * eops.P.v[r] + eops.ps * eops.R.v[r], h.v[r]);
            }
            qw_tail<O, EPI, GW, NSLOT>(cam, gl, slot, active, h, a, eops, red);
            return;
        }
    }
    qw_finish<O, EPI, GW, NSLOT>(cam, gl, slot, active, acc, alpha, a, eops, red);
}

bool sell_supports(int o) { return o == 1 || (o >= 3 && o <= 5); }
void sell_quat_roundtrip(const double block[9], double quat[4], double rebuilt[9]) {
    double b[9], q[4], r[9];
    for (int e = 0; e < 9; ++e) b[e] = block[e];
    block_to_quat(b, q);
    quat_to_block(q[0], q[1], q[2], q[3], r);
    for (int e = 0; e < 4; ++e) quat[e] = q[e];
    for (int e = 0; e < 9; ++e) rebuilt[e] = r[e];
}

template <int O>
static void qw_sell_o(int epi, SellMatrix &m, const double *W, double alpha, const CamArgs &a, int gm, hipStream_t st, const double *Wpad16) {
    const TcgScal *sc = (epi == EPI_HESS) ? a.scal : (const TcgScal *)nullptr;
    double *parts = m.parts(O);
    SellArgs sa = m.args();
    sa.wstride = m.wstride(O);
    const bool quat = m.codec() == SELL_CODEC_QUAT;
    const bool padded = Wpad16 != nullptr && O >= 3 && 3 * pitch_of(O) <= 16;
    const double *Wn = W;
    const int wn = sa.wstride;
    if (padded) { sa.wstride = 16; W = Wpad16; }
    if (m.grid() > 0) {
        const dim3 g(m.grid()), b(256);
        if (gm != 0 && (uint64_t)m.ncols() * (uint64_t)sa.wstride * 8u >= (1ull << 32)) gm = 0;
        sa.nt_off = m.nt_off(O, a.nloc);
        if (quat) {
            if constexpr (O == 3) {
                if (gm == 1) hipLaunchKernelGGL((qw_sell_kernel_q_occ4<1>), g, b, 0, st, sa, W, sc, parts);
                else hipLaunchKernelGGL((qw_sell_kernel_q_occ4<0>), g, b, 0, st, sa, W, sc, parts);
            } else {
                if (gm == 1) hipLaunchKernelGGL((qw_sell_kernel<O, 1, 0, SELL_CODEC_QUAT>), g, b, 0, st, sa, W, sc, parts);
                else hipLaunchKernelGGL((qw_sell_kernel<O, 0, 0, SELL_CODEC_QUAT>), g, b, 0, st, sa, W, sc, parts);
            }
        } else {
            constexpr int PIPE = (O == 3) ? 1 : 0;
            if (gm == 1) hipLaunchKernelGGL((qw_sell_kernel<O, 1, PIPE>), g, b, 0, st, sa, W, sc, parts);
            else hipLaunchKernelGGL((qw_sell_kernel<O, 0, PIPE>), g, b, 0, st, sa, W, sc, parts);
        }
    }
    const dim3 g(m.reduce_grid(O, a.nloc)), b(256);
#define XM_SELL_REDUCE(GW_)                                                                                                                          \
    switch (epi) {                                                                                                                                  \
        case EPI_PLAIN: hipLaunchKernelGGL((sell_reduce_kernel<O, EPI_PLAIN, GW_>), g, b, 0, st, sa.pptr, sa.ridx, parts, alpha, a, sa.diag, Wn, sa.row0, wn); break; \
        case EPI_GRAD: hipLaunchKernelGGL((sell_reduce_kernel<O, EPI_GRAD, GW_>), g, b, 0, st, sa.pptr, sa.ridx, parts, alpha, a, sa.diag, Wn, sa.row0, wn); break;   \
        case EPI_HESS: hipLaunchKernelGGL((sell_reduce_kernel<O, EPI_HESS, GW_>), g, b, 0, st, sa.pptr, sa.ridx, parts, alpha, a, sa.diag, Wn, sa.row0, wn); break;   \
        default: throw Error(XM_ERR_ARG, "bad epilogue");                                                                                           \
    }
    if (m.reduce_gw(O) == 4) { XM_SELL_REDUCE(4) } else { XM_SELL_REDUCE(16) }
#undef XM_SELL_REDUCE
}

void launch_qw_sell(int o, int epi, SellMatrix &m, const double *W, double alpha, const CamArgs &a, int gm, hipStream_t st, const double *Wpad16) {
    if (a.nloc <= 0) return;
    if (epi == EPI_CERT) {
        if (o != 1) throw Error(XM_ERR_ARG, "certificate operator needs o == 1");
        double *parts = m.parts(1);
        SellArgs sa = m.args();
        sa.wstride = 3;
        if (m.grid() > 0) {
            sa.nt_off = m.nt_off(1, a.nloc);
            if (m.codec() == SELL_CODEC_QUAT) hipLaunchKernelGGL((qw_sell_kernel<1, 0, 0, SELL_CODEC_QUAT>), dim3(m.grid()), dim3(256), 0, st, sa, W, (const TcgScal *)nullptr, parts);
            else hipLaunchKernelGGL((qw_sell_kernel<1, 0>), dim3(m.grid()), dim3(256), 0, st, sa, W, (const TcgScal *)nullptr, parts);
        }
        if (m.reduce_gw(1) == 4) hipLaunchKernelGGL((sell_reduce_kernel<1, EPI_CERT, 4>), dim3(m.reduce_grid(1, a.nloc)), dim3(256), 0, st, sa.pptr, sa.ridx, parts, alpha, a, sa.diag, W, sa.row0, sa.wstride);
        else hipLaunchKernelGGL((sell_reduce_kernel<1, EPI_CERT, 16>), dim3(m.reduce_grid(1, a.nloc)), dim3(256), 0, st, sa.pptr, sa.ridx, parts, alpha, a, sa.diag, W, sa.row0, sa.wstride);
    } else {
        switch (o) {
            case 1: qw_sell_o<1>(epi, m, W, alpha, a, 0, st, nullptr); break;
            case 3: qw_sell_o<3>(epi, m, W, alpha, a, gm, st, Wpad16); break;
            case 4: qw_sell_o<4>(epi, m, W, alpha, a, gm, st, Wpad16); break;
            case 5: qw_sell_o<5>(epi, m, W, alpha, a, gm, st, Wpad16); break;
            default: throw Error(XM_ERR_ARG, "SELL product is instantiated for o = 1, 3, 4, 5");
        }
    }
    check_launch("qw_sell");
}

}
```

xm-code_amd/csrc/xm_solver.h:

```cpp
#pragma once

#include <chrono>
#include <cstdint>
#include <cstdio>
#include <memory>
#include <string>
#include <vector>

#include "../../include/xm_amd.h"
#include "xm_common.h"

namespace xm {

struct Settings {
    int sym = 0;
    int64_t sym_min_rows = 0;
    int64_t sym_rows(int world) const { return sym_min_rows > 0 ? sym_min_rows : (world <= 1 ? 4096 : 6144); }
    int sell = 0;
    int sell_slabs = 4, sell_lmax = 64, sell_gather = 1;
    int sell_codec = 0;
    int sell_wpad = 0;
    int overlap = 0;
    double overlap_min_mb = 64.0;
    int64_t cert_dense_rows = 384;
// ... 146 lines not shown
    int64_t n_landmarks() const;
    void dense_q(double *q, int64_t ldq);
    bool schur_info(int64_t out[3], double *relres) const;
    int schur_precond(int64_t *aggregates, int *block) const;

private:
    int64_t n_ = 0;
    int nloc_ = 0;
    int cam0_ = 0;
    int64_t g0_ = 0;
    int64_t true_loc_ = 0;
    int64_t ntot_ = 0;
    int64_t ld_ = 0;
    int storage_ = XM_STORAGE_DENSE;
    double *dQ_ = nullptr;
    bool ownQ_ = false;
    float *dQ32_ = nullptr;
    void refresh_q32();
    DevBuf<double> Afull_;
    DevBuf<int64_t> rowptr_;
    DevBuf<int32_t> colidx_;
    DevBuf<double> blocks_;
    int64_t nb_loc_ = 0;
    DevBuf<int4> rowinfo_;
    std::unique_ptr<SellMatrix> sell_;
    int sell_gm_ = 0;
    std::unique_ptr<SchurOp> schur_;
    bool schur_dense_ = false;
    int64_t ne_ = 0;
    DevBuf<int32_t> ei_, ej_, inc_edge_;
    DevBuf<int64_t> inc_ptr_, pos_ij_, pos_ji_, pos_d_;
    DevBuf<double> eM_, ew_, eres_;
    bool solved_ = false;
    std::vector<double> w_cur_;
    DevBuf<double> eerr_;
    const double *residuals_recovered_device(const double *rot, const double *scale);
    hipStream_t st_ = nullptr;
    hipStream_t st2_ = nullptr;
    hipEvent_t ev_w_ = nullptr, ev_p_ = nullptr;
    DevBuf<double> Pstrip_;
    bool w_pending_ = false;
    std::shared_ptr<Comm> comm_;
    Settings cfg_;
    PeerXchg xchg_;
    double *partsB_peer_ = nullptr;
    unsigned long long tcg_runs_ = 0;
    std::vector<int64_t> cam_cut_;
    int retraction_ = 0, grouping_ = 0;

    int o_ = 0, OP_ = 0;
    DevBuf<double> R_, s_, Rc_, sc_, W_, D_;
    DevBuf<double> wpad_;
    double *wpad() const { return (wpad_.p && wpad_on_) ? wpad_.p : nullptr; }
    bool wpad_on_ = false;
    const double *wpad_next_ = nullptr;
    PointState ps_[2];
    int cur_ = 0;
    DevBuf<double> rR_, rs_, rsB_, pR_, psA_, psB_, vR_, vs_, HvR_, Hvs_, HpR_, Hps_;
    DevBuf<double> partsA_, partsB_, partsM_;
    DevBuf<double> Prow_, Pcol_;
    DevBuf<double> ksum_;
    DevBuf<unsigned int> kcount_;
    int ks_ = 1;
    std::unique_ptr<SymwProduct> symw_;
    void product_symw(int epi, int o, double alpha, const CamArgs &a);
    bool sym_ok_ = false;
    int sym_max_o_ = 4;
    bool eig_exact_ = false;
    double q_asym_ = 0, q_max_ = 0;
    DevBuf<TcgScal> scal_;
    unsigned long long *hstat_ = nullptr;
    unsigned long long *hstat_dev_ = nullptr;
    double *hpin_ = nullptr;
    double *hpin_dev_ = nullptr;
    size_t hpin_count_ = 0;
    int nA_ = 0, nB_ = 0;
    unsigned long long outer_seq_ = 0;

    const xm_options_t *opt_ = nullptr;
    xm_result_t *res_ = nullptr;
    bool verbose_ = false;
    std::vector<std::pair<hipEvent_t, hipEvent_t>> ev_pool_;
    size_t ev_used_ = 0;
    int64_t hess_launches_ = 0;
    int sym_rev_ = 1;
    std::vector<float> qw_samples_;

    void init(const xm_problem_t &prob);
    void to_host(void *dst, const void *src_dev, size_t bytes);
    void to_dev(void *dst_dev, const void *src, size_t bytes);
    void ensure_pinned(size_t doubles);
    DevBuf<double> lzV_, lzc_, lzw_, lzc2_, lzab_, lzscr_;
    DevBuf<double> recW_;
    int64_t pos_of(int64_t g) const;
    void release_raw();
    void setup_rank(int o);
    void upload_point(const std::vector<double> &R_cm, int o, const std::vector<double> &s_ex);
    void download_point(std::vector<double> &R_cm, std::vector<double> &s_ex);
    CamArgs cam_args(int state) const;
    int prod_grid() const;
    int tcg_blocks() const;
    void product(int epi, int o, double alpha, const CamArgs &a);
    void gather_W();
    void flush_gather();
    bool overlap_applies() const;
    void eval_point(int state, const double *Rp, const double *sp, double &f, double &rr);
    double sum_parts(const double *dparts, int count);
    int run_tcg(double rr, double delta, TcgScal &fin, int adopted = 0);
    int enqueue_spec_tcg();
    void tcg_enqueue_iteration(int i, bool profile);
    bool spec_applies() const;
    DevBuf<SpecCtl> spec_;
    unsigned int tcg_seq_ = 0;
    volatile double *wait_outer_result();
    bool stream_idle(std::chrono::steady_clock::time_point t_wait, const char *what);
    bool agree_any(bool local);
    void drain_events();
    void finish_profile();
    TrResult trust_region(int o, double &gradtol, double linesearch_step, const std::vector<double> &v_dir, double max_time);
    bool device_outer_applies(int o) const;
    TrResult trust_region_device(int o, double &gradtol, double f, double rr, double delta, double delta_bar, double max_time);
    DevBuf<double> trace_dev_;
    DevBuf<int> stop_req_;
    DevBuf<OuterScal> oscal_;
    unsigned int outer_run_ = 0;
    CertResult certificate(int o, double primal, std::vector<double> &v_out);
    int lanczos_min(std::vector<double> &x_out, double &theta, int &iters, double &resid);
    void cert_product(const double *vj, const CamArgs &a, int j);
    void log(const char *fmt, ...) const;
};

class Team {
public:
    Team(const xm_problem_t &prob, int n_gpus, int gpu_map);
    ~Team();
    Team(const Team &) = delete;
    Team &operator=(const Team &) = delete;
    int world() const;
    int comm_kind() const;
    int product_kind(int o) const;
    const std::string &fallback_note() const;
    void solve(const xm_options_t &opt, xm_result_t &res);
    void attach_edges(int64_t ne, const int32_t *ei, const int32_t *ej, const double *M);
    void edge_residuals(double *res);
    void set_edge_weights(const double *w);
    void edge_residuals_recovered(const double *rot, const double *scale, double *res);
    double xm2_filter(const double *rot, const double *scale, double pct, int64_t *removed, double *w_out);
    int64_t cameras() const;
    std::vector<double> weights() const;
private:
    struct Impl;
    std::unique_ptr<Impl> p_;
    void shutdown();
};

}
```

xm-code_amd/csrc/xm_solver.hip:

```cpp
#include "xm_solver.h"
#include "xm_sell.h"
#include "xm_symw.h"
#include "xm_schur.h"
#include "xm_ba.h"
#include "xm_clean.h"

#include <algorithm>
#include <chrono>
#include <cmath>
#include <cstdarg>
#include <cstdlib>
#include <cstring>
#include <thread>

namespace xm {

using clk = std::chrono::steady_clock;
static double secs_since(clk::time_point t0) { return std::chrono::duration<double>(clk::now() - t0).count(); }

void Context::log(const char *fmt, ...) const {
    if (!verbose_ || (comm_ && comm_->rank != 0)) return;
    va_list ap;
    va_start(ap, fmt);
    vprintf(fmt, ap);
// ... 379 lines not shown
            XM_HIP_CHECK(hipMemcpyAsync(repd.p + (size_t)rank * 2, mine2, sizeof(mine2), hipMemcpyHostToDevice, st_));
            comm_->allgather(repd.p, 2, st_);
            std::vector<unsigned long long> all((size_t)world * 2);
            XM_HIP_CHECK(hipMemcpyAsync(all.data(), repd.p, all.size() * sizeof(unsigned long long), hipMemcpyDeviceToHost, st_));
            XM_HIP_CHECK(hipStreamSynchronize(st_));
            unsigned long long tot = 0ull, bad2 = 0ull;
            for (int r = 0; r < world; ++r) { tot += all[(size_t)2 * r]; bad2 |= all[(size_t)2 * r + 1]; }
            if (tot != 0ull || bad2 != 0ull) symw_.reset();
        }
        comm_->host_barrier();
    }
    XM_HIP_CHECK(hipHostMalloc((void **)&hstat_, 256, hipHostMallocMapped | hipHostMallocCoherent));
    std::memset(hstat_, 0, 256);
    XM_HIP_CHECK(hipHostGetDevicePointer((void **)&hstat_dev_, hstat_, 0));
    ensure_pinned((size_t)1 << 17);
    if (viewgraph) {
        attach_edges(prob.ne, prob.edge_i, prob.edge_j, prob.edge_M);
        w_cur_.assign(prob.edge_w, prob.edge_w + prob.ne);
    }
}

Context::~Context() { release_raw(); }

void Context::setup_rank(int o) {
    if (comm_->active()) comm_->host_barrier();
    o_ = o;
    OP_ = pitch_of(o);
    const size_t mat = (size_t)nloc_ * 3 * OP_, vec = (size_t)nloc_;
    const int world = comm_->world;
    const int o_top = std::max(o, (int)std::min<unsigned>(opt_ ? opt_->max_rank : 0u, (unsigned)kMaxRank));
    const size_t mat_top = (size_t)nloc_ * 3 * pitch_of(o_top);
    for (DevBuf<double> *b : {&R_, &Rc_, &D_, &rR_, &pR_, &vR_, &HvR_, &HpR_}) b->ensure(mat, st_, mat_top);
    for (DevBuf<double> *b : {&s_, &sc_, &rs_, &rsB_, &psA_, &psB_, &vs_, &Hvs_, &Hps_}) b->ensure(vec, st_);
    for (int k = 0; k < 2; ++k) {
        ps_[k].G.ensure(mat, st_, mat_top); ps_[k].rgR.ensure(mat, st_, mat_top); ps_[k].egs.ensure(vec, st_); ps_[k].rgs.ensure(vec, st_); ps_[k].S0.ensure(vec * 9, st_);
    }
    cur_ = 0;
    wpad_on_ = sell_ && cfg_.sell_wpad >= 0 && !comm_->active() && sell_supports(o) && o >= 3 && 3 * OP_ <= 16 && (cfg_.sell_wpad == 1 || sell_->padded_pays(o));
    if (wpad_on_ && !wpad_.p) wpad_.alloc((size_t)ntot_ * 16 + 16);
    W_.ensure((size_t)ld_ * OP_ + 16, st_, (size_t)ld_ * pitch_of(o_top) + 16);
    const int nA_loc = prod_grid(), nB_loc = tcg_blocks();
    nA_ = nA_loc * world;
    nB_ = nB_loc * world;
    partsA_.ensure((size_t)3 * nA_, st_);
    const size_t b_off = comm_->active() ? mat : 0;
    const size_t pb = (size_t)2 * (b_off * world + 3 * nA_ + nB_);
    if (comm_->peer() && world > 1 && cfg_.exchange != 1 && !symw_ && storage_ != XM_STORAGE_SCHUR && comm_->device_waits()) {
        partsB_.release();
        comm_->xchg_setup(pb, xchg_);
        partsB_peer_ = xchg_.buf[comm_->rank];
        xchg_.mute = (cfg_.debug_peer_mute && comm_->rank == 1) ? 1 : 0;
        xchg_.lite = cfg_.exchange_lite;
    } else {
        xchg_ = PeerXchg();
        partsB_peer_ = nullptr;
        partsB_.ensure(pb, st_, (size_t)2 * ((comm_->active() ? mat_top : 0) * world + 3 * nA_ + nB_));
    }
    if (comm_->active()) Afull_.ensure(mat * world, st_, mat_top * world); else Afull_.release();
    partsM_.ensure((size_t)std::max(std::max(nB_, flat_grid((int64_t)mat_top) * world), 4 * ((nloc_ + 255) / 256) * world), st_);
    if (sym_ok_ && o >= 3 && o <= sym_max_o_) {
        Prow_.alloc(sym_prow_count(nloc_, ld_, o));
        Pcol_.alloc(sym_pcol_count(nloc_, ld_, o), false);
    } else {
        Prow_.release(); Pcol_.release();
    }
    ks_ = 1;
    if (storage_ == XM_STORAGE_DENSE && !sym_ok_ && cfg_.split_k >= 0) {
        if (cfg_.split_k >= 2) ks_ = std::min(cfg_.split_k, std::max(1, (int)((ld_ + 255) / 256)));
        else if (comm_->active()) ks_ = qw_dense_split_k(nloc_, ld_);
    }
    if (ks_ > 1) {
        ksum_.alloc((size_t)ks_ * mat);
        kcount_.alloc((size_t)qw_grid(nloc_));
    }
    if (overlap_applies()) {
        if (!st2_) {
            XM_HIP_CHECK(hipStreamCreateWithFlags(&st2_, hipStreamNonBlocking));
            XM_HIP_CHECK(hipEventCreateWithFlags(&ev_w_, hipEventDisableTiming));
            XM_HIP_CHECK(hipEventCreateWithFlags(&ev_p_, hipEventDisableTiming));
        }
        Pstrip_.alloc(mat);
    }
    scal_.ensure(2, st_);
    spec_.ensure(1, st_);
    if (sell_ && sell_supports(o)) (void)sell_->parts(o);
    ensure_pinned(std::max<size_t>((size_t)2 * nA_ + (size_t)nB_ + partsM_.count + 64, (size_t)ld_ * OP_ + (size_t)ntot_ + 1024));
    if (comm_->active()) comm_->host_barrier();
}

void Context::upload_point(const std::vector<double> &R_cm, int o, const std::vector<double> &s_ex) {
    const size_t m = (size_t)3 * n_;
    std::vector<double> Rr((size_t)nloc_ * 3 * OP_, 0.0), sl((size_t)nloc_, 1.0);
    for (int c = 0; c < nloc_; ++c) {
        const bool real = c < true_loc_;
        const int64_t g = g0_ + c;
        for (int a = 0; a < 3; ++a)
            for (int k = 0; k < o; ++k)
                Rr[((size_t)c * 3 + a) * OP_ + k] = real ? R_cm[(size_t)(3 * g + a) + (size_t)k * m] : (a == k ? 1.0 : 0.0);
        if (real) sl[(size_t)c] = s_ex[(size_t)g];
    }
    if (cam0_ == 0) sl[0] = 1.0;
    to_dev(R_.p, Rr.data(), Rr.size() * sizeof(double));
    to_dev(s_.p, sl.data(), sl.size() * sizeof(double));
}

void Context::download_point(std::vector<double> &R_cm, std::vector<double> &s_ex) {
    const size_t m = (size_t)3 * n_, mat = (size_t)nloc_ * 3 * OP_;
    std::vector<double> full((size_t)ntot_ * 3 * OP_), sf((size_t)ntot_);
    launch_scale_copy(W_.p + (size_t)comm_->rank * mat, R_.p, 1.0, (int64_t)mat, st_);
    if (comm_->active()) comm_->allgather(W_.p, mat, st_);
    to_host(full.data(), W_.p, full.size() * sizeof(double));
    launch_scale_copy(W_.p + (size_t)comm_->rank * nloc_, s_.p, 1.0, (int64_t)nloc_, st_);
    if (comm_->active()) comm_->allgather(W_.p, (size_t)nloc_, st_);
    to_host(sf.data(), W_.p, sf.size() * sizeof(double));
    XM_HIP_CHECK(hipMemsetAsync(W_.p, 0, W_.count * sizeof(double), st_));
    R_cm.assign(m * (size_t)o_, 0.0);
    s_ex.assign((size_t)n_, 1.0);
    for (int64_t g = 0; g < n_; ++g) {
        const size_t q = (size_t)pos_of(g);
        for (int a = 0; a < 3; ++a)
            for (int k = 0; k < o_; ++k) R_cm[(size_t)(3 * g + a) + (size_t)k * m] = full[(q * 3 + a) * OP_ + k];
        s_ex[(size_t)g] = sf[q];
    }
}

int Context::prod_grid() const {
    if (storage_ == XM_STORAGE_BSR3 && sell_ && sell_supports(o_)) return sell_->reduce_grid(o_, nloc_);
    return (storage_ == XM_STORAGE_BSR3) ? bsr_grid(nloc_) : qw_grid(nloc_);
}

int Context::tcg_blocks() const {
    int g = flat_grid((int64_t)nloc_ * 3 * OP_);
    if (comm_->peer() && comm_->world > 1 && cfg_.exchange != 1 && !symw_ && storage_ != XM_STORAGE_SCHUR && comm_->device_waits()) g = std::min(g, std::max(8, 1024 / std::max(1, comm_->ranks_on_my_device())));
    return g;
}

CamArgs Context::cam_args(int state) const {
    CamArgs a;
    std::memset(&a, 0, sizeof(a));
    a.nloc = nloc_;
    a.cam0 = cam0_;
    a.lam = opt_ ? opt_->lam : 0.0;
    a.R = R_.p;
    a.s = s_.p;
    const PointState &p = ps_[state];
    a.G = p.G.p; a.egs = p.egs.p; a.S0 = p.S0.p; a.rgR = p.rgR.p; a.rgs = p.rgs.p;
    a.pR = pR_.p; a.ps = psA_.p; a.rR = rR_.p; a.rs = rs_.p; a.HpR = HpR_.p; a.Hps = Hps_.p;
    a.Wloc = W_.p + (size_t)cam0_ * 3 * OP_;
    a.out = HpR_.p;
    a.partials = partsA_.p;
    a.scal = scal_.p;
    if (ks_ > 1) { a.ks = ks_; a.ksum = ksum_.p; a.kcount = kcount_.p; }
    return a;
}

void Context::product(int epi, int o, double alpha, const CamArgs &a) {
    if (w_pending_) {
        if (storage_ == XM_STORAGE_DENSE && (epi == EPI_PLAIN || epi == EPI_GRAD) && o == o_) {
            w_pending_ = false;
            const int tc = qw_dense_tile_cols();
            const int64_t c0 = 3 * (int64_t)cam0_, c1 = 3 * ((int64_t)cam0_ + nloc_);
            CamArgs s1 = a, s2 = a;
            s1.range_mode = 1; s1.t_lo = (int)((c0 + tc - 1) / tc); s1.t_hi = (int)(c1 / tc); s1.out = Pstrip_.p; s1.addend = nullptr;
            s2.range_mode = 2; s2.t_lo = s1.t_lo; s2.t_hi = s1.t_hi; s2.addend = Pstrip_.p;
            comm_->note("overlap_split", (double)s1.t_lo, (double)s1.t_hi);
            XM_HIP_CHECK(hipEventRecord(ev_w_, st_));
            XM_HIP_CHECK(hipStreamWaitEvent(st2_, ev_w_, 0));
            launch_qw_dense_split(o, EPI_PLAIN, dQ_, ld_, W_.p, 1.0, s1, st2_);
            XM_HIP_CHECK(hipEventRecord(ev_p_, st2_));
            comm_->allgather(W_.p, (size_t)nloc_ * 3 * OP_, st_);
            XM_HIP_CHECK(hipStreamWaitEvent(st_, ev_p_, 0));
            launch_qw_dense_split(o, epi, dQ_, ld_, W_.p, alpha, s2, st_);
            if (res_) res_->qw_products++;
            return;
        }
        flush_gather();
    }
    if (storage_ == XM_STORAGE_DENSE && dQ32_ && o == o_ && (epi == EPI_HESS || epi == EPI_AUTO)) {
        if (sym_ok_ && o >= 3 && o <= sym_max_o_ && Pcol_.p) launch_qw_sym_f32(o, epi, dQ32_, dQ_, ld_, W_.p, alpha, a, Prow_.p, Pcol_.p, st_, sym_rev_);
        else { CamArgs ar = a; ar.rev = sym_rev_; launch_qw_dense_f32(o, epi, dQ32_, dQ_, ld_, W_.p, alpha, ar, st_); }
    } else if (storage_ == XM_STORAGE_DENSE) {
        if (symw_ && o == o_ && o >= 3 && o <= sym_max_o_ && epi != EPI_CERT) product_symw(epi, o, alpha, a);
        else if (sym_ok_ && o == o_ && o >= 3 && o <= sym_max_o_ && epi != EPI_CERT && Pcol_.p) launch_qw_sym(o, epi, dQ_, ld_, W_.p, alpha, a, Prow_.p, Pcol_.p, st_, sym_rev_);
        else { CamArgs ar = a; ar.rev = sym_rev_; launch_qw_dense(o, epi, dQ_, ld_, W_.p, alpha, ar, st_); }
    } else if (storage_ == XM_STORAGE_SCHUR) {
        schur_->product(o, epi, W_.p, alpha, a, st_);
    } else if (sell_ && sell_supports(o)) {
        const double *wp = (epi == EPI_HESS && o == o_) ? wpad() : ((epi == EPI_GRAD && o == o_) ? wpad_next_ : nullptr);
        wpad_next_ = nullptr;
        launch_qw_sell(o, epi, *sell_, W_.p, alpha, a, sell_gm_, st_, wp);
    } else {
        launch_qw_bsr3(o, epi, rowptr_.p, colidx_.p, blocks_.p, W_.p, alpha, a, st_, nb_loc_, rowinfo_.p);
    }
    if (res_) res_->qw_products++;
}

int Context::product_kind(int o) const {
    if (storage_ == XM_STORAGE_SCHUR) return XM_PRODUCT_SCHUR;
    if (storage_ == XM_STORAGE_DENSE) return ((symw_ || sym_ok_) && o >= 3 && o <= sym_max_o_) ? XM_PRODUCT_DENSE_SYM : XM_PRODUCT_DENSE;
    if (sell_ && sell_supports(o)) return sell_->codec() == SELL_CODEC_QUAT ? XM_PRODUCT_SELL_QUAT : XM_PRODUCT_SELL;
    return XM_PRODUCT_BSR3;
}

void Context::product_symw(int epi, int o, double alpha, const CamArgs &a) {
    symw_->sweep(o, dQ_, W_.p, (epi == EPI_HESS) ? a.scal : (const TcgScal *)nullptr, comm_->rank, st_);
    comm_->allgather(symw_->csum_all(), symw_->csum_count(o), st_);
    symw_->reduce(o, epi, alpha, a, comm_->world, st_);
}

bool Context::overlap_applies() const {
    if (cfg_.overlap < 0 || !comm_->active() || storage_ != XM_STORAGE_DENSE || sym_ok_ || symw_) return false;
    if ((double)nloc_ * 3.0 * (double)ld_ * 8.0 < cfg_.overlap_min_mb * 1048576.0) return false;
    const int tc = qw_dense_tile_cols();
    const int64_t c0 = 3 * (int64_t)cam0_, c1 = 3 * ((int64_t)cam0_ + nloc_);
    return (c1 / tc) > ((c0 + tc - 1) / tc);
}

void Context::gather_W() {
    if (!comm_->active()) return;
    if (overlap_applies()) { w_pending_ = true; return; }
    comm_->allgather(W_.p, (size_t)nloc_ * 3 * OP_, st_);
}

void Context::flush_gather() {
    if (!w_pending_) return;
    w_pending_ = false;
    comm_->allgather(W_.p, (size_t)nloc_ * 3 * OP_, st_);
}

double Context::sum_parts(const double *dparts, int count) {
    if (comm_->peer()) launch_copy_words(hpin_dev_, dparts, (size_t)count * sizeof(double), st_);
    else XM_HIP_CHECK(hipMemcpyAsync(hpin_, dparts, (size_t)count * sizeof(double), hipMemcpyDeviceToHost, st_));
    XM_HIP_CHECK(hipStreamSynchronize(st_));
    double t = 0.0;
    for (int i = 0; i < count; ++i) t += hpin_[i];
    return t;
}

void Context::eval_point(int state, const double *Rp, const double *sp, double &f, double &rr) {
    const int nA_loc = prod_grid();
    CamArgs a = cam_args(state);
    a.R = Rp;
    a.s = sp;
    a.partials = partsA_.p + (size_t)comm_->rank * 2 * nA_loc;
    product(EPI_GRAD, o_, 2.0, a);
    if (comm_->active()) comm_->allgather(partsA_.p, (size_t)2 * nA_loc, st_);
    launch_outer_finalize(partsA_.p, nA_loc, comm_->world, partsM_.p, 0, scal_.p, reinterpret_cast<double *>(hstat_dev_) + 8,
                          ++outer_seq_, grouping_, st_);
    volatile double *hres = wait_outer_result();
    f = hres[0];
    rr = hres[1];
}

bool Context::agree_any(bool local) {
    if (!comm_->active()) return local;
    const int world = comm_->world;
    double v = local ? 1.0 : 0.0;
    to_dev(partsM_.p + comm_->rank, &v, sizeof(double));
    comm_->allgather(partsM_.p, 1, st_);
    if (comm_->peer()) launch_copy_words(hpin_dev_, partsM_.p, (size_t)world * sizeof(double), st_);
    else XM_HIP_CHECK(hipMemcpyAsync(hpin_, partsM_.p, (size_t)world * sizeof(double), hipMemcpyDeviceToHost, st_));
    XM_HIP_CHECK(hipStreamSynchronize(st_));
    bool any = false;
    for (int r = 0; r < world; ++r) any = any || (hpin_[r] != 0.0);
    return any;
}

bool Context::stream_idle(clk::time_point t_wait, const char *what) {
    const double limit = cfg_.watchdog_s;
    comm_->check_device_error();
    const hipError_t q = hipStreamQuery(st_);
    if (q == hipSuccess) return true;
    if (q != hipErrorNotReady) {
        (void)hipGetLastError();
        throw Error(XM_ERR_HIP, std::string("device error while waiting for ") + what + ": " + hipGetErrorString(q));
    }
    if (secs_since(t_wait) > limit)
        throw Error(XM_ERR_HIP, std::string("watchdog: no progress for ") + std::to_string((int)limit) + " s while waiting for " + what);
    return false;
}

volatile double *Context::wait_outer_result() {
    volatile unsigned long long *hseq = reinterpret_cast<volatile unsigned long long *>(hstat_) + 8 + 5;
    const unsigned long long seq = outer_seq_;
    const auto t_wait = clk::now();
    auto t_check = t_wait;
    while (*hseq != seq) {
        __builtin_ia32_pause();
        if (secs_since(t_check) > 500e-6) {
            if (stream_idle(t_wait, "the outer-iteration results")) {
                XM_HIP_CHECK(hipStreamSynchronize(st_));
                if (*hseq != seq) throw Error(XM_ERR_HIP, "outer-iteration results did not reach host-mapped memory");
            }
            t_check = clk::now();
        }
    }
    return reinterpret_cast<volatile double *>(hstat_) + 8;
}

void Context::drain_events() {
    for (size_t i = 0; i < ev_used_; ++i) {
        float ms = 0.f;
        if (hipEventElapsedTime(&ms, ev_pool_[i].first, ev_pool_[i].second) == hipSuccess) qw_samples_.push_back(ms);
    }
    ev_used_ = 0;
}

void Context::finish_profile() {
    drain_events();
    if (qw_samples_.empty()) return;
    std::vector<float> v = qw_samples_;
    std::sort(v.begin(), v.end());
    const float ref = v[(v.size() * 3) / 4];
    for (float x : v)
        if (x >= 0.5f * ref) { res_->qw_ms_sum += x; res_->qw_ms_count++; }
    qw_samples_.clear();
}

void Context::tcg_enqueue_iteration(int i, bool profile) {
    const int nA_loc = prod_grid(), nB_loc = tcg_blocks();
    const int rank = comm_->rank;
    const bool fused = xchg_.world > 1;
    const bool lockstep = comm_->active() && !fused;
    double *Wloc = wpad() ? nullptr : W_.p + (size_t)cam0_ * 3 * OP_;
    const int par = i & 1;
    CamArgs a = cam_args(cur_);
    a.scal = scal_.p + par;
    a.ps = par ? psB_.p : psA_.p;
    a.rs = par ? rsB_.p : rs_.p;
    const size_t mat = (size_t)nloc_ * 3 * OP_;
    const size_t b_off = comm_->active() ? mat : 0;
    const size_t chunk = b_off + (size_t)3 * nA_loc + nB_loc;
    double *pB = fused ? partsB_peer_ : partsB_.p;
    double *pcur = pB + (size_t)par * chunk * comm_->world, *pnext = pB + (size_t)(par ^ 1) * chunk * comm_->world;
    a.partials = pcur + (size_t)rank * chunk + b_off;
    a.Bout = comm_->active() ? pcur + (size_t)rank * chunk : nullptr;
    const bool timed = profile && (hess_launches_ % kProfileStride == 0) && ev_used_ < ev_pool_.size();
    if (timed) XM_HIP_CHECK(hipEventRecord(ev_pool_[ev_used_].first, st_));
    const bool model_rec = opt_ && (opt_->flags & XM_FLAG_MODEL_RECURRENCE);
    sym_rev_ = par;
    product(EPI_HESS, o_, 2.0, a);
    sym_rev_ = 1;
    if (timed) { XM_HIP_CHECK(hipEventRecord(ev_pool_[ev_used_].second, st_)); ev_used_++; }
    hess_launches_++;
    if (lockstep) comm_->allgather(pcur, chunk, st_);
    launch_cg_step(o_, nloc_, scal_.p + par, scal_.p + (par ^ 1), pcur, nA_loc, nB_loc, comm_->world, HpR_.p, Hps_.p, R_.p,
                   s_.p, pR_.p, par ? psB_.p : psA_.p, par ? psA_.p : psB_.p, vR_.p, vs_.p, model_rec ? nullptr : HvR_.p, model_rec ? nullptr : Hvs_.p, rR_.p,
                   par ? rsB_.p : rs_.p, par ? rs_.p : rsB_.p, Wloc, pnext + (size_t)rank * chunk + b_off + 3 * nA_loc, hstat_dev_,
                   (int)b_off, (int64_t)mat, comm_->active() ? Afull_.p : nullptr, W_.p, grouping_, xchg_, st_, wpad());
}

bool Context::spec_applies() const {
    return !comm_->active() && opt_ && !(opt_->flags & XM_FLAG_HOST_STEPPED) && storage_ != XM_STORAGE_SCHUR && cfg_.debug_drop_finalize < 0;
}

int Context::enqueue_spec_tcg() {
    std::swap(R_.p, Rc_.p);
    std::swap(s_.p, sc_.p);
    cur_ ^= 1;
    const PointState &P = ps_[cur_];
    double *Wloc = wpad() ? nullptr : W_.p + (size_t)cam0_ * 3 * OP_;
    ++tcg_seq_;
    launch_tcg_init(o_, nloc_, P.rgR.p, P.rgs.p, R_.p, s_.p, rR_.p, rs_.p, pR_.p, psA_.p, vR_.p, vs_.p, HvR_.p, Hvs_.p, Wloc,
                    scal_.p, 0.0, 0.0, hstat_dev_, st_, wpad(), (int)tcg_seq_, spec_.p);
    const int n_spec = 1;
    for (int i = 0; i < n_spec; ++i) tcg_enqueue_iteration(i, false);
    std::swap(R_.p, Rc_.p);
    std::swap(s_.p, sc_.p);
    cur_ ^= 1;
    return n_spec;
}

int Context::run_tcg(double rr, double delta, TcgScal &fin, int adopted) {
    const bool stepped = (opt_->flags & XM_FLAG_HOST_STEPPED) != 0;
    const bool profile = (opt_->flags & XM_FLAG_PROFILE_QW) != 0;
    double *Wloc = wpad() ? nullptr : W_.p + (size_t)cam0_ * 3 * OP_;
    const PointState &P = ps_[cur_];
    if (comm_->active()) comm_->note("tcg_start", rr, delta);
    if (adopted == 0) {
        ++tcg_seq_;
        launch_tcg_init(o_, nloc_, P.rgR.p, P.rgs.p, R_.p, s_.p, rR_.p, rs_.p, pR_.p, psA_.p, vR_.p, vs_.p, HvR_.p, Hvs_.p, Wloc,
                        scal_.p, rr, delta, hstat_dev_, st_, wpad(), (int)tcg_seq_);
        gather_W();
    }
    const bool fused = xchg_.world > 1;
    if (fused) xchg_.epoch_base = (++tcg_runs_) << 12;
    const bool lockstep = comm_->active() && !fused;
    const int run_ahead = (lockstep || prod_grid() >= 64) ? 2 : 3;
    int fin_status = 0, fin_iter = 0;
    int it = adopted;
    auto enqueue = [&](int i) { tcg_enqueue_iteration(i, profile); };
    auto read_scal = [&](int par) {
        TcgScal sc;
        to_host(&sc, scal_.p + par, sizeof(TcgScal));
        return sc;
    };
    if (stepped) {
        for (;;) {
            TcgScal sc = read_scal(it & 1);
            if (sc.status != 0 || it >= kMaxInner) break;
            enqueue(it++);
        }
    } else {
        volatile unsigned long long *hs = hstat_;
        auto last_progress = clk::now();
        auto last_change = last_progress;
        unsigned long long seen = ~0ull;
        for (;;) {
            const unsigned long long v = *hs;
            if (v != seen) { seen = v; last_progress = clk::now(); last_change = last_progress; }
            const bool valid = (unsigned int)(v >> 32) == tcg_seq_;
            const int status = valid ? (int)(v & 0xff) : 0;
            const int done = valid ? (int)((v >> 8) & 0xffffff) : 0;
            if (status != 0) { fin_status = status; fin_iter = done; break; }
            if (it < kMaxInner && it - done < run_ahead) { enqueue(it++); continue; }
            __builtin_ia32_pause();
            if (secs_since(last_progress) > 200e-6) {
                if (stream_idle(last_change, "the truncated-CG progress word")) {
                    TcgScal sc = read_scal(it & 1);
                    if (sc.status != 0) { fin_status = sc.status; fin_iter = sc.iter; break; }
                    if (it >= kMaxInner) { fin_status = 6; fin_iter = kMaxInner; break; }
                    *hstat_ = ((unsigned long long)tcg_seq_ << 32) | ((unsigned long long)(unsigned)sc.iter << 8);
                    if (it - sc.iter >= run_ahead) enqueue(it++);
                }
                last_progress = clk::now();
            }
        }
    }
    if (comm_->active()) comm_->note("tcg_end_before_topup", (double)it, (double)(fin_iter * 16 + fin_status));
    if (fin_status == 7) { comm_->check_device_error(); throw Error(XM_ERR_COMM, "peer exchange: a rank did not arrive inside the truncated CG"); }
    if (lockstep && !stepped) {
        const int T = (fin_status == 6) ? fin_iter - 1 : fin_iter;
        while (it < std::min(kMaxInner, T + 2)) enqueue(it++);
    }
    (void)fin;
    return it;
}

TrResult Context::trust_region(int o, double &gradtol, double linesearch_step, const std::vector<double> &v_dir, double max_time) {
    TrResult out;
    const double dim = (double)n_ * (3.0 * o - 6.0) + (double)n_ - 1.0;
    const double delta_bar = std::sqrt(dim);
    double delta = delta_bar / 8.0;
    double *Wloc = W_.p + (size_t)cam0_ * 3 * OP_;
    double f = 0, rr = 0;

    log("start linesearch\n");
    if (linesearch_step != 0) {
        launch_scale_rows(o, nloc_, R_.p, s_.p, Wloc, st_);
        gather_W();
        double f0, tmp;
        eval_point(cur_ ^ 1, R_.p, s_.p, f0, tmp);
        double alpha = linesearch_step;
        std::vector<double> D((size_t)nloc_ * 3 * OP_, 0.0);
        for (int c = 0; c < (int)true_loc_; ++c) {
            const int64_t g = g0_ + c;
            for (int a = 0; a < 3; ++a) D[((size_t)c * 3 + a) * OP_ + (o - 1)] = v_dir[(size_t)(3 * g + a)];
        }
        to_dev(D_.p, D.data(), D.size() * sizeof(double));
        double fn;
        for (;;) {
            launch_retract(o, nloc_, cam0_, R_.p, s_.p, D_.p, nullptr, -alpha, Rc_.p, nullptr, Wloc, st_, retraction_);
            gather_W();
            eval_point(cur_ ^ 1, Rc_.p, s_.p, fn, tmp);
            if (!(fn > f0)) break;
            alpha *= 0.5;
            if (alpha < 1e-20) { log("linesearch failed! BM stopped! \n"); out.primal = -1; out.ls_failed = true; out.stop_reason = -1; return out; }
        }
        if (f0 - fn > 0) {
            log("linesearch decrease %1.3e\n", f0 - fn);
            if (opt_->flags & XM_FLAG_FIX_STALE_SR) {
                std::swap(R_.p, Rc_.p);
                launch_scale_rows(o, nloc_, R_.p, s_.p, Wloc, st_);
            } else {
                launch_scale_rows(o, nloc_, R_.p, s_.p, Wloc, st_);
                std::swap(R_.p, Rc_.p);
            }
            gather_W();
        } else {
            log("linesearch failed! BM stopped! \n");
            out.primal = -1; out.ls_failed = true; out.stop_reason = -1;
            return out;
        }
    } else {
        launch_scale_rows(o, nloc_, R_.p, s_.p, Wloc, st_);
        gather_W();
    }
    eval_point(cur_, R_.p, s_.p, f, rr);
    if (device_outer_applies(o)) return trust_region_device(o, gradtol, f, rr, delta, delta_bar, max_time);
    double loss = f;

    int endreason = 6, trstatus = 4, shrink_count = 0, inner_print = 1, k = 0;
    int adopted = 0;
    long long totalite = 0;
    int stop_reason = 14;
    const auto start = clk::now();
    for (k = 0; k < kMaxOuter; ++k) {
        const double gradnorm = std::sqrt(rr);
        if (verbose_) {
            static const char *trn[] = {"", "TR- ", "TR+ ", "REJ ", "TR "};
            if (k > 0) log("%s", trn[trstatus]);
            log("%d   %d   %1.3e   %1.3e", k, inner_print, loss, gradnorm);
            if (k > 0) {
                const char *er = endreason == 1 ? "nagative curvature" : endreason == 2 ? "exceed trust region"
                               : endreason == 3 ? "reached norm tolerance" : endreason == 5 ? "numerical issue" : "max iteration";
                log("   %s\n", er);
            } else log("\n");
        }
        if (opt_->trace && res_->trace_len < opt_->trace_cap) {
            double *tr = opt_->trace + (size_t)res_->trace_len * 6;
            tr[0] = loss; tr[1] = gradnorm; tr[2] = inner_print; tr[3] = endreason; tr[4] = trstatus; tr[5] = delta;
            res_->trace_len++;
        }
        if (endreason == 5) { stop_reason = 5; log("Terminate because of rdotr touched machine precise\n"); break; }
        if (gradnorm < gradtol) { log("Terminate because of small gradient norm\n"); gradtol /= 10; stop_reason = 10; break; }
        if (agree_any((double)(long long)secs_since(start) > max_time)) { log("Terminate because of time limit\n"); stop_reason = 11; break; }
        endreason = 6; trstatus = 4;

        TcgScal fin;
        const int enq = run_tcg(rr, delta, fin, adopted);
        adopted = 0;

        const int nA_loc = prod_grid();
        const PointState &P = ps_[cur_];
        const int nB_loc = retract_grid(nloc_);
        const bool model_rec = (opt_->flags & XM_FLAG_MODEL_RECURRENCE) != 0;
        launch_retract_model(o, nloc_, cam0_, R_.p, s_.p, vR_.p, vs_.p, Rc_.p, sc_.p, Wloc, wpad(), model_rec ? nullptr : HvR_.p, Hvs_.p, P.rgR.p, P.rgs.p,
                             partsM_.p + (size_t)comm_->rank * nB_loc, st_, retraction_ == XM_RETRACT_POLAR ? 1 : 0);
        if (comm_->active() && !model_rec) comm_->allgather(partsM_.p, (size_t)nB_loc, st_);
        gather_W();
        wpad_next_ = wpad();
        {
            CamArgs a = cam_args(cur_ ^ 1);
            a.R = Rc_.p;
            a.s = sc_.p;
            a.partials = partsA_.p + (size_t)comm_->rank * 2 * nA_loc;
            product(EPI_GRAD, o_, 2.0, a);
            if (comm_->active()) comm_->allgather(partsA_.p, (size_t)2 * nA_loc, st_);
        }
        const long long drop_at = cfg_.debug_drop_finalize;
        const bool spec = spec_applies();
        const OuterArgs oa = {loss, delta, delta_bar, gradtol, shrink_count, (k + 1 >= kMaxOuter) ? 1 : 0};
        if (drop_at >= 0 && (long long)outer_seq_ + 1 == drop_at) ++outer_seq_;
        else
        launch_outer_finalize(partsA_.p, nA_loc, comm_->world, partsM_.p, model_rec ? 0 : nB_loc * comm_->world, scal_.p + (enq & 1),
                              reinterpret_cast<double *>(hstat_dev_) + 8, ++outer_seq_, grouping_, st_, spec ? &oa : nullptr, spec_.p);
        const int n_spec = spec ? enqueue_spec_tcg() : 0;
        volatile double *hres = wait_outer_result();
        double f_new = hres[0], rr_new = hres[1], loss_qu = hres[2];
        const bool spec_go = spec && hres[6] != 0.0;
        const double spec_delta = hres[7];
        fin.status = (int)hres[3];
        fin.iter = (int)hres[4];
        if (fin.status == 7) { comm_->check_device_error(); throw Error(XM_ERR_COMM, "peer exchange: a rank did not arrive inside the truncated CG"); }
        if (fin.status == 0) fin.status = 6;
        endreason = fin.status;
        inner_print = fin.iter + 1;
        totalite += fin.iter + 1;
        if (opt_->flags & XM_FLAG_PROFILE_QW) drain_events();
        if (loss_qu >= 0) { log("error! loss_qu is larger than 0\n"); stop_reason = 12; break; }
        const double rou = (f_new - loss) / loss_qu;
        if (rou < 0.25) { delta *= 0.25; trstatus = 1; shrink_count++; }
        else if (rou > 0.75 && endreason <= 2) { delta = std::min(delta * 2, delta_bar); trstatus = 2; shrink_count = 0; }
        else shrink_count = 0;
        bool stop_delta = false;
        if (shrink_count > 3) {
            delta *= 1e-3; shrink_count = 0;
            log("delta shrinked to %1.3e\n", delta);
            if (delta < 1e-20) { log("delta is too small, BM stopped!\n"); stop_delta = true; }
        }
        const bool reject = (f_new > loss || rou < 0.1);
        if (stop_delta || !reject) {
            std::swap(R_.p, Rc_.p);
            std::swap(s_.p, sc_.p);
            cur_ ^= 1;
            if (stop_delta) { stop_reason = 13; break; }
            loss = f_new;
            rr = rr_new;
            if (spec_go && std::memcmp(&spec_delta, &delta, sizeof(double)) == 0) adopted = n_spec;
        } else {
            trstatus = 3;
        }
        if (n_spec > 0 && adopted != n_spec && res_) res_->qw_products -= n_spec;
    }
    log("\nTotal iteration:     %lld\n", totalite);
    const double secs = secs_since(start);
    log("Time taken by function1: %lld ms\n", (long long)(secs * 1e3));
    res_->tcg_iters += totalite;
    res_->outer_iters += k;
    res_->tr_seconds += secs;
    res_->last_stop_reason = stop_reason;
    out.primal = loss;
    out.outer_iters = k;
    out.stop_reason = stop_reason;
    return out;
}

bool Context::device_outer_applies(int o) const {
    if (!opt_ || (opt_->flags & (XM_FLAG_HOST_OUTER | XM_FLAG_HOST_STEPPED))) return false;
    if (comm_->active() || symw_ || storage_ == XM_STORAGE_SCHUR || o < 3 || cfg_.debug_drop_finalize >= 0) return false;
    if (storage_ == XM_STORAGE_BSR3 && sell_ && sell_supports(o)) return false;
    if (storage_ == XM_STORAGE_DENSE && ks_ > 1) return false;
    if (storage_ == XM_STORAGE_DENSE && !(opt_->flags & XM_FLAG_DEVICE_OUTER)) return false;
    return true;
}

TrResult Context::trust_region_device(int o, double &gradtol, double f, double rr, double delta, double delta_bar, double max_time) {
    TrResult out;
    const auto start = clk::now();
    const bool profile = (opt_->flags & XM_FLAG_PROFILE_QW) != 0;
    const bool model_rec = (opt_->flags & XM_FLAG_MODEL_RECURRENCE) != 0;
    const int nA = prod_grid(), nB = tcg_blocks(), nM = retract_grid(nloc_);
    double loss = f;
    int stop_reason = 14, k = 0;
    long long totalite = 0;
    int trace0 = res_->trace_len;
    if (opt_->trace && res_->trace_len < opt_->trace_cap) {
        double *tr = opt_->trace + (size_t)res_->trace_len * 6;
        tr[0] = loss; tr[1] = std::sqrt(rr); tr[2] = 1; tr[3] = 6; tr[4] = 4; tr[5] = delta;
        res_->trace_len++;
    }
    auto progress_line = [&](int kk, const double *rec, double delta_prev) {
        static const char *trn[] = {"", "TR- ", "TR+ ", "REJ ", "TR "};
        const int er = (int)rec[3], ts = (int)rec[4];
        if (kk > 0 && rec[5] < delta_prev * 0.25 * 0.5) log("delta shrinked to %1.3e\n", rec[5]);
        if (kk > 0) log("%s", trn[(ts >= 0 && ts <= 4) ? ts : 0]);
        log("%d   %d   %1.3e   %1.3e", kk, (int)rec[2], rec[0], rec[1]);
        if (kk > 0) log("   %s\n", er == 1 ? "nagative curvature" : er == 2 ? "exceed trust region" : er == 3 ? "reached norm tolerance" : er == 5 ? "numerical issue" : "max iteration");
        else log("\n");
    };
    {
        const double rec0[6] = {loss, std::sqrt(rr), 1, 6, 4, delta};
        progress_line(0, rec0, delta);
    }
    bool run = true;
    if (std::sqrt(rr) < gradtol) { stop_reason = 10; run = false; }
    else if ((double)(long long)secs_since(start) > max_time) { stop_reason = 11; run = false; }
    long long slots_live = 0, slots_enq = 0;
    if (run) {
        if (trace_dev_.count < (size_t)kMaxOuter * 6) trace_dev_.alloc((size_t)kMaxOuter * 6);
        if (stop_req_.count < 1) stop_req_.alloc(1);
        XM_HIP_CHECK(hipMemsetAsync(stop_req_.p, 0, sizeof(int), st_));
        if (oscal_.count < 2) oscal_.alloc(2);
        TcgScal init;
        std::memset(&init, 0, sizeof(init));
        init.phase = PH_INIT; init.delta = delta; init.seq = (int)++tcg_seq_;
        OuterScal oinit;
        std::memset(&oinit, 0, sizeof(oinit));
        oinit.loss = loss; oinit.rr_point = rr;
        to_dev(scal_.p + 1, &init, sizeof(init));
        to_dev(oscal_.p + 1, &oinit, sizeof(oinit));
        const unsigned int runid = ++outer_run_;
        volatile unsigned long long *hp = hstat_ + 24;
        *hp = 0;
        const size_t chunk = (size_t)3 * nA + nB;
        double *Wloc = W_.p + (size_t)cam0_ * 3 * OP_;
        const PointState &Pc = ps_[cur_], &Pn = ps_[cur_ ^ 1];
        auto step_args = [&](int slot) {
            const int par = slot & 1;
            OuterStepArgs A;
            std::memset(&A, 0, sizeof(A));
            A.nloc = nloc_; A.cam0 = cam0_;
            A.scal_cur = scal_.p + par; A.scal_next = scal_.p + (par ^ 1);
            A.os_cur = oscal_.p + par; A.os_next = oscal_.p + (par ^ 1);
            A.parts = partsB_.p + (size_t)par * chunk;
            A.partsB_out = partsB_.p + (size_t)(par ^ 1) * chunk + (size_t)3 * nA;
// ... 755 lines not shown
    xm::reprojection_errors(*schur_, rot, t, p, sqerr, cfg_.watchdog_s, st_);
}
void Context::clean_observations(const CleanSettings &cfg, uint8_t *keep, int32_t *cam_index, int32_t *lm_index, CleanOutcome &out) {
    if (!schur_)
        throw Error(XM_ERR_ARG, "xm_ctx_clean_observations: needs a matrix-free context (XM_STORAGE_SCHUR): the other storages hold no observations");
    if (comm_->active()) throw Error(XM_ERR_ARG, "xm_ctx_clean_observations: single-rank contexts only");
    CleanSettings c = cfg;
    c.watchdog_s = cfg_.watchdog_s;
    xm::clean_observations(*schur_, c, keep, cam_index, lm_index, out, st_);
}
void Context::dense_q(double *q, int64_t ldq) {
    if (!schur_dense_ || !dQ_) throw Error(XM_ERR_ARG, "xm_ctx_dense_q: the context holds no dense Q built from observations (xm_tuning_t.schur_dense_q)");
    if (!q || ldq < 3 * n_) throw Error(XM_ERR_ARG, "xm_ctx_dense_q: null output or ldq < 3n");
    XM_HIP_CHECK(hipMemcpy2DAsync(q, (size_t)ldq * sizeof(double), dQ_, (size_t)ld_ * sizeof(double), (size_t)3 * n_ * sizeof(double), (size_t)3 * n_,
                                  hipMemcpyDeviceToHost, st_));
    XM_HIP_CHECK(hipStreamSynchronize(st_));
}
int64_t Context::n_landmarks() const { return schur_ ? schur_->n_landmarks() : 0; }
bool Context::schur_info(int64_t out[3], double *relres) const {
    if (!schur_ || !schur_->uses_pcg()) return false;
    schur_->pcg_stats(out, relres);
    return true;
}
int Context::schur_precond(int64_t *aggregates, int *block) const {
    *aggregates = 0; *block = 0;
    if (!schur_ || !schur_->uses_pcg()) return -1;
    if (!schur_->two_level()) return 0;
    *aggregates = schur_->aggregates(); *block = kSchurAggCams;
    return 1;
}

void Context::refresh_q32() {
    const size_t rows = (size_t)3 * nloc_;
    if (!dQ32_) XM_HIP_CHECK(hipMalloc((void **)&dQ32_, rows * (size_t)ld_ * sizeof(float)));
    DevBuf<unsigned int> bad;
    bad.alloc(1);
    launch_dense_to_f32(dQ_, dQ32_, (int64_t)rows, ld_, bad.p, st_);
    unsigned int h = 0;
    XM_HIP_CHECK(hipMemcpyAsync(&h, bad.p, sizeof(h), hipMemcpyDeviceToHost, st_));
    XM_HIP_CHECK(hipStreamSynchronize(st_));
    if (h) throw Error(XM_ERR_ARG, "xm_tuning_t.hess_f32: " + std::to_string(h) + " entries of Q are not finite in fp32");
}

void Context::set_edge_weights(const double *w) {
    if (schur_) {
        schur_->set_weights(w, st_);
        w_cur_.assign(w, w + schur_->nobs());
        if (schur_dense_) {
            schur_->build_dense_q(dQ_, ld_, nullptr, st_);
            if (dQ32_) refresh_q32();
        }
        return;
    }
    if (!ei_.p) throw Error(XM_ERR_ARG, "set_edge_weights: no edges attached");
    if (ne_ > 0 && !w) throw Error(XM_ERR_ARG, "set_edge_weights: null weights");
    w_cur_.assign(w, w + ne_);
    if (ne_ > 0) to_dev(ew_.p, w, (size_t)ne_ * sizeof(double));
    const bool dense = (storage_ == XM_STORAGE_DENSE);
    launch_edge_write(dense, ne_, ei_.p, ej_.p, eM_.p, ew_.p, cam0_, nloc_, inc_ptr_.p, inc_edge_.p, pos_ij_.p, pos_ji_.p, pos_d_.p,
                      dense ? nullptr : blocks_.p, dense ? dQ_ : nullptr, ld_, st_);
    if (sell_) sell_->refill(colidx_.p, blocks_.p, st_);
    if (dQ32_) refresh_q32();
    XM_HIP_CHECK(hipStreamSynchronize(st_));
}

void Context::solve(const xm_options_t &opt, xm_result_t &res) {
    opt_ = &opt;
    res_ = &res;
    verbose_ = (opt.flags & XM_FLAG_VERBOSE) != 0;
    if (opt.retraction != XM_RETRACT_QR && opt.retraction != XM_RETRACT_POLAR) throw Error(XM_ERR_ARG, "unknown retraction");
    if (opt.sum_grouping < 0 || opt.sum_grouping > 2) throw Error(XM_ERR_ARG, "sum_grouping must be 0, 1 or 2");
    retraction_ = opt.retraction;
    grouping_ = opt.sum_grouping;
    double *Rout = res.R, *sout = res.s;
    std::memset(&res, 0, sizeof(res));
    res.R = Rout; res.s = sout;
    if (!Rout || !sout) throw Error(XM_ERR_ARG, "result buffers missing");
    if (opt.max_rank > (unsigned)kMaxRank) throw Error(XM_ERR_ARG, "max_rank > 10 is not instantiated");
    if ((opt.flags & XM_FLAG_PROFILE_QW) && ev_pool_.empty()) {
        ev_pool_.resize(256);
        for (auto &e : ev_pool_) { XM_HIP_CHECK(hipEventCreate(&e.first)); XM_HIP_CHECK(hipEventCreate(&e.second)); }
    }
    ev_used_ = 0;
    hess_launches_ = 0;
    qw_samples_.clear();
    const auto t0 = clk::now();
    const size_t m = (size_t)3 * n_;
    log("+++++++++++++++++++++++++++++++++\nBegin XM\n+++++++++++++++++++++++++++++++++\n");
    unsigned o = 3;
    std::vector<double> v(m, 0.0), R0(m * 3, 0.0), Rk, s0((size_t)n_, 1.0), sk;
    if (opt.mode == XM_MODE_REBUTTLE && opt.s_ini) for (int64_t i = 0; i < n_; ++i) s0[(size_t)i] = opt.s_ini[i];
    const double s_anchor = s0[0];
    double gradtol = opt.tol, primal = 0;
    int status = XM_STATUS_NONE;
    auto identity_stack = [&]() {
        R0.assign(m * 3, 0.0);
        for (size_t i = 0; i < (size_t)n_; ++i) { R0[3 * i] = 1.0; R0[3 * i + m + 1] = 1.0; R0[3 * i + 2 * m + 2] = 1.0; }
    };
    int out_rank = 3;
    if (opt.mode == XM_MODE_RANK3) {
        log("+++++++++++++++++++++++++++++++++\nSolve TR with Rank   3\n+++++++++++++++++++++++++++++++++\n");
        identity_stack();
        setup_rank(3);
        upload_point(R0, 3, s0);
        TrResult tr = trust_region(3, gradtol, 0.0, v, opt.max_time);
        primal = tr.primal;
        download_point(R0, s0);
        out_rank = 3;
    } else {
        while (o <= opt.max_rank) {
            log("+++++++++++++++++++++++++++++++++\nSolve TR with Rank   %u\n+++++++++++++++++++++++++++++++++\n", o);
            TrResult tr;
            setup_rank((int)o);
            if (o == 3) {
                identity_stack();
                if ((opt.flags & XM_FLAG_WARM_R) && !opt.R_ini) throw Error(XM_ERR_ARG, "XM_FLAG_WARM_R without R_ini");
                const bool warm = (opt.flags & XM_FLAG_WARM_R) && opt.R_ini;
                if (warm) std::memcpy(R0.data(), opt.R_ini, m * 3 * sizeof(double));
                upload_point(R0, 3, s0);
                if (warm) {
                    XM_HIP_CHECK(hipMemsetAsync(D_.p, 0, D_.count * sizeof(double), st_));
                    launch_retract(3, nloc_, cam0_, R_.p, s_.p, D_.p, nullptr, 0.0, Rc_.p, nullptr, nullptr, st_, 0);
                    std::swap(R_.p, Rc_.p);
                }
                tr = trust_region(3, gradtol, 0.0, v, opt.max_time);
            } else {
                upload_point(R0, (int)o, s0);
                tr = trust_region((int)o, gradtol, 1.0, v, opt.max_time);
            }
            primal = tr.primal;
            if (primal < 0) { status = XM_STATUS_LS_FAILED; o += 1; break; }
            log("+++++++++++++++++++++++++++++++++\nCheck Eigen value\n+++++++++++++++++++++++++++++++++\n");
            CertResult ce = certificate((int)o, primal, v);
            res.dual = ce.dual; res.min_eig = ce.min_eig; res.gap = ce.gap;
            download_point(Rk, sk);
            if (ce.accepted) {
                R0 = Rk; s0 = sk; o += 1; status = XM_STATUS_CERTIFIED;
                break;
            } else if (o < opt.max_rank) {
                R0.assign(m * (o + 1), 0.0);
                std::copy(Rk.begin(), Rk.end(), R0.begin());
                s0 = sk;
                for (size_t i = 0; i < (size_t)n_; ++i) { v[3 * i] /= sk[i]; v[3 * i + 1] /= sk[i]; v[3 * i + 2] /= sk[i]; }
            } else {
                R0 = Rk; s0 = sk; status = XM_STATUS_MAX_RANK;
            }
            o += 1;
        }
        if (o > opt.max_rank) log("BM stoped because max rank\n");
        out_rank = (int)o - 1;
    }
    res.rank = out_rank;
    if (out_rank >= 3 && R0.size() >= m * (size_t)out_rank) std::memcpy(Rout, R0.data(), m * (size_t)out_rank * sizeof(double));
    for (int64_t i = 0; i < n_; ++i) sout[i] = s0[(size_t)i];
    sout[0] = s_anchor;
    res.status = status;
    res.primal = primal;
    if (opt.flags & XM_FLAG_PROFILE_QW) finish_profile();
    const int of = std::max(3, std::min(out_rank, (int)opt.max_rank));
    res.sym_product = ((sym_ok_ || symw_) && storage_ == XM_STORAGE_DENSE) ? 1 : 0;
    res.hess_f32 = dQ32_ ? 1 : 0;
    const int64_t qel = dQ32_ ? 4 : 8;
    if (storage_ == XM_STORAGE_DENSE) res.qw_bytes = qel * (3 * n_) * (3 * n_) + 2LL * 8 * 3 * n_ * of;
    else if (storage_ == XM_STORAGE_SCHUR) res.qw_bytes = schur_->bytes_per_product(of);
    else res.qw_bytes = 76LL * nb_loc_ + 4LL * (n_ + 1) + 2LL * 8 * 3 * n_ * of;
    res.qw_stream_bytes = (storage_ == XM_STORAGE_DENSE) ? (symw_ ? symw_->stream_bytes() : (res.sym_product ? qel / 2 : qel) * (3 * n_) * (3 * n_))
// ... 11 lines not shown
```

Measured before the change: 24470.

## Fuse outer finalize with speculative tCG init and split Hessian product launches

Merges the outer trust-region finalize reduction and the speculative tCG init into one kernel. Every block makes the accept decision, and the last block to arrive writes the next scalar state through an atomic counter. It also splits each Hessian-vector iteration into a product half and a reduce/CG-step half, so the host can enqueue the next product ahead of the current step's completion check. This cuts launch count and host-device latency between outer and inner iterations, at the cost of more complex queue-depth bookkeeping and a grid-wide arrival counter.

```diff
diff --git a/xm-code_amd/csrc/xm_common.h b/xm-code_amd/csrc/xm_common.h
--- a/xm-code_amd/csrc/xm_common.h
+++ b/xm-code_amd/csrc/xm_common.h
@@ -182,12 +182,12 @@
                           int grid[2], hipStream_t st);
 void symv_plan_get(int nloc, int64_t ld, int out[4]);
 void launch_qw_sym(int o, int epi, const double *Q, int64_t ld, const double *W, double alpha, const CamArgs &a, double *Prow,
-                   double *Pcol, hipStream_t st, int rev = 0);
+                   double *Pcol, hipStream_t st, int rev = 0, int part = 0);
 void launch_asym(const double *Q, int64_t ld, int64_t m, double *out, int grid, hipStream_t st);
 void launch_dense_to_f32(const double *src, float *dst, int64_t rows, int64_t ld, unsigned int *bad, hipStream_t st);
 void launch_qw_dense_f32(int o, int epi, const float *Qf, const double *Qd, int64_t ld, const double *W, double alpha, const CamArgs &a, hipStream_t st);
 void launch_qw_sym_f32(int o, int epi, const float *Qf, const double *Qd, int64_t ld, const double *W, double alpha, const CamArgs &a, double *Prow,
-                       double *Pcol, hipStream_t st, int rev = 0);
+                       double *Pcol, hipStream_t st, int rev = 0, int part = 0);
 
 void launch_symhash(const double *Q, int64_t ld, int64_t row0, int64_t nrows, int64_t m, unsigned long long *out, int grid, hipStream_t st);
 
@@ -200,16 +200,19 @@
 void launch_scale_rows(int o, int nloc, const double *R, const double *s, double *Wloc, hipStream_t st);
 void launch_tcg_init(int o, int nloc, const double *rgR, const double *rgs, const double *R, const double *s, double *rR,
                      double *rs, double *pR, double *ps, double *vR, double *vs, double *HvR, double *Hvs, double *Wloc,
-                     TcgScal *scal0, double rr, double delta, unsigned long long *hstat, hipStream_t st, double *Wpad = nullptr, int seq = 0,
-                     const SpecCtl *spec = nullptr);
+                     TcgScal *scal0, double rr, double delta, unsigned long long *hstat, hipStream_t st, double *Wpad = nullptr, int seq = 0);
 void launch_cg_step(int o, int nloc, const TcgScal *scal_cur, TcgScal *scal_next, const double *parts, int nA_loc, int nB_loc, int world,
                     const double *HpR, const double *Hps, const double *R, const double *s, double *pR,
                     const double *ps_cur, double *ps_next, double *vR, double *vs, double *HvR, double *Hvs, double *rR, const double *rs_cur,
                     double *rs_next, double *Wloc, double *partsB_out, unsigned long long *hstat, int b_off, int64_t mat, double *Afull,
                     double *Wfull, int grouping, const struct PeerXchg &xchg, hipStream_t st, double *Wpad = nullptr);
 struct OuterArgs { double loss, delta, delta_bar, gradtol; int shrink_count, last_iter; };
+struct OuterSums { const double *partsA; int nA; const double *partsM; int nM; const TcgScal *scal_fin; double *hres; unsigned long long seq; int grouping; };
+void launch_tcg_start(int o, int nloc, const double *rgR, const double *rgs, const double *R, const double *s, double *rR, double *rs,
+                      double *pR, double *ps, double *vR, double *vs, double *HvR, double *Hvs, double *Wloc, TcgScal *scal0,
+                      unsigned long long *hstat, hipStream_t st, double *Wpad, int seq, const OuterSums &os, const OuterArgs &oa, unsigned int *arrive);
 void launch_outer_finalize(const double *partsA, int nA_loc, int world, const double *partsM, int nM, const TcgScal *scal, double *hres,
-                           unsigned long long seq, int grouping, hipStream_t st, const OuterArgs *oa = nullptr, SpecCtl *spec_out = nullptr);
+                           unsigned long long seq, int grouping, hipStream_t st);
 void launch_retract(int o, int nloc, int cam0, const double *R, const double *s, const double *D, const double *ds, double t,
                     double *Rout, double *sout, double *Wloc, hipStream_t st, int polar = 0);
 int retract_grid(int nloc);
diff --git a/xm-code_amd/csrc/xm_kernels.hip b/xm-code_amd/csrc/xm_kernels.hip
--- a/xm-code_amd/csrc/xm_kernels.hip
+++ b/xm-code_amd/csrc/xm_kernels.hip
@@ -849,20 +849,11 @@
 }
 
 template <int O>
-__global__ __launch_bounds__(256) void tcg_init_kernel(int nloc, const double *__restrict__ rgR, const double *__restrict__ rgs,
-                                                        const double *__restrict__ R, const double *__restrict__ s,
-                                                        double *rR, double *rs, double *pR, double *ps, double *vR, double *vs,
-                                                        double *HvR, double *Hvs, double *Wloc, TcgScal *scal0, double rr,
-                                                        double delta, unsigned long long *hstat, double *Wpad, int seq, const SpecCtl *spec) {
+__device__ __forceinline__ void tcg_init_vectors(int nloc, const double *__restrict__ rgR, const double *__restrict__ rgs,
+                                                 const double *__restrict__ R, const double *__restrict__ s, double *rR, double *rs, double *pR,
+                                                 double *ps, double *vR, double *vs, double *HvR, double *Hvs, double *Wloc, double *Wpad) {
     constexpr int OP = pitch_of(O);
     const int64_t total = (int64_t)nloc * 3 * OP;
-    if (spec != nullptr) {
-        if (!spec->go) {
-            if (blockIdx.x == 0 && threadIdx.x == 0) { TcgScal sc = *scal0; sc.status = 9; sc.seq = seq; *scal0 = sc; }
-            return;
-        }
-        rr = spec->rr; delta = spec->delta;
-    }
     for (int64_t i = (int64_t)blockIdx.x * 256 + threadIdx.x; i < total; i += (int64_t)gridDim.x * 256) {
         const int cam = (int)(i / (3 * OP));
         const double g = rgR[i], gs = rgs[cam];
@@ -872,6 +863,14 @@
         if (Wpad) Wpad[(size_t)cam * 16 + (i - (int64_t)cam * (3 * OP))] = wv;
         if (i % (3 * OP) == 0) { rs[cam] = gs; ps[cam] = -gs; vs[cam] = 0.0; Hvs[cam] = 0.0; }
     }
+}
+template <int O>
+__global__ __launch_bounds__(256) void tcg_init_kernel(int nloc, const double *__restrict__ rgR, const double *__restrict__ rgs,
+                                                        const double *__restrict__ R, const double *__restrict__ s,
+                                                        double *rR, double *rs, double *pR, double *ps, double *vR, double *vs,
+                                                        double *HvR, double *Hvs, double *Wloc, TcgScal *scal0, double rr,
+                                                        double delta, unsigned long long *hstat, double *Wpad, int seq) {
+    tcg_init_vectors<O>(nloc, rgR, rgs, R, s, rR, rs, pR, ps, vR, vs, HvR, Hvs, Wloc, Wpad);
     if (blockIdx.x == 0 && threadIdx.x == 0) {
         TcgScal sc = {};
         sc.rr = rr; sc.vv = 0.0; sc.vp = 0.0; sc.pp = rr; sc.delta = delta; sc.gradnorm = sqrt(rr); sc.last_step = 0.0; sc.model = 0.0;
@@ -1102,10 +1101,43 @@
     }
 }
 
+__device__ __forceinline__ SpecCtl tr_decide(double f, double rr, double m, const TcgScal &sc, const OuterArgs &oa) {
+    const int endreason = (sc.status == 0) ? 6 : sc.status;
+    double delta = oa.delta;
+    int shrink = oa.shrink_count;
+    bool go = (m < 0.0) && endreason != 7;
+    if (go) {
+        const double rou = (f - oa.loss) / m;
+        if (rou < 0.25) { delta *= 0.25; shrink++; }
+        else if (rou > 0.75 && endreason <= 2) { delta = fmin(delta * 2, oa.delta_bar); shrink = 0; }
+        else shrink = 0;
+        bool stop_delta = false;
+        if (shrink > 3) { delta *= 1e-3; shrink = 0; if (delta < 1e-20) stop_delta = true; }
+        const bool reject = (f > oa.loss || rou < 0.1);
+        go = !stop_delta && !reject && endreason != 5 && !(sqrt(rr) < oa.gradtol) && !oa.last_iter;
+    }
+    SpecCtl sp;
+    sp.go = go ? 1 : 0; sp.pad_ = 0; sp.rr = rr; sp.delta = delta;
+    return sp;
+}
+__device__ __forceinline__ void publish_outer_result(double *hres, double f, double rr, double m, const TcgScal &sc, const SpecCtl *sp,
+                                                     unsigned long long seq) {
+    __hip_atomic_store(hres + 0, f, __ATOMIC_RELAXED, __HIP_MEMORY_SCOPE_SYSTEM);
+    __hip_atomic_store(hres + 1, rr, __ATOMIC_RELAXED, __HIP_MEMORY_SCOPE_SYSTEM);
+    __hip_atomic_store(hres + 2, m, __ATOMIC_RELAXED, __HIP_MEMORY_SCOPE_SYSTEM);
+    __hip_atomic_store(hres + 3, (double)sc.status, __ATOMIC_RELAXED, __HIP_MEMORY_SCOPE_SYSTEM);
+    __hip_atomic_store(hres + 4, (double)sc.iter, __ATOMIC_RELAXED, __HIP_MEMORY_SCOPE_SYSTEM);
+    if (sp != nullptr) {
+        __hip_atomic_store(hres + 6, sp->go ? 1.0 : 0.0, __ATOMIC_RELAXED, __HIP_MEMORY_SCOPE_SYSTEM);
+        __hip_atomic_store(hres + 7, sp->delta, __ATOMIC_RELAXED, __HIP_MEMORY_SCOPE_SYSTEM);
+    }
+    __atomic_thread_fence(__ATOMIC_SEQ_CST);
+    asm volatile("s_waitcnt vmcnt(0)" ::: "memory");
+    __hip_atomic_store(reinterpret_cast<unsigned long long *>(hres + 5), seq, __ATOMIC_RELEASE, __HIP_MEMORY_SCOPE_SYSTEM);
+}
 __global__ __launch_bounds__(256) void outer_finalize_kernel(const double *__restrict__ partsA, int nA_loc, int world,
                                                               const double *__restrict__ partsM, int nM,
-                                                              const TcgScal *__restrict__ scal, double *hres, unsigned long long seq, int grp,
-                                                              OuterArgs oa, SpecCtl *spec_out) {
+                                                              const TcgScal *__restrict__ scal, double *hres, unsigned long long seq, int grp) {
     __shared__ double sh[4];
     double f = 0.0, rr = 0.0;
     for (int r = 0; r < world; ++r) {
@@ -1116,36 +1148,49 @@
     if (threadIdx.x == 0) {
         const TcgScal sc = *scal;
         const double m = (nM > 0) ? m_vec : sc.model;
-        __hip_atomic_store(hres + 0, f, __ATOMIC_RELAXED, __HIP_MEMORY_SCOPE_SYSTEM);
-        __hip_atomic_store(hres + 1, rr, __ATOMIC_RELAXED, __HIP_MEMORY_SCOPE_SYSTEM);
-        __hip_atomic_store(hres + 2, m, __ATOMIC_RELAXED, __HIP_MEMORY_SCOPE_SYSTEM);
-        __hip_atomic_store(hres + 3, (double)sc.status, __ATOMIC_RELAXED, __HIP_MEMORY_SCOPE_SYSTEM);
-        __hip_atomic_store(hres + 4, (double)sc.iter, __ATOMIC_RELAXED, __HIP_MEMORY_SCOPE_SYSTEM);
-        if (spec_out != nullptr) {
-            const int endreason = (sc.status == 0) ? 6 : sc.status;
-            double delta = oa.delta;
-            int shrink = oa.shrink_count;
-            bool go = (m < 0.0) && endreason != 7;
-            if (go) {
-                const double rou = (f - oa.loss) / m;
-                if (rou < 0.25) { delta *= 0.25; shrink++; }
-                else if (rou > 0.75 && endreason <= 2) { delta = fmin(delta * 2, oa.delta_bar); shrink = 0; }
-                else shrink = 0;
-                bool stop_delta = false;
-                if (shrink > 3) { delta *= 1e-3; shrink = 0; if (delta < 1e-20) stop_delta = true; }
-                const bool reject = (f > oa.loss || rou < 0.1);
-                go = !stop_delta && !reject && endreason != 5 && !(sqrt(rr) < oa.gradtol) && !oa.last_iter;
-            }
-            SpecCtl sp;
-            sp.go = go ? 1 : 0; sp.pad_ = 0; sp.rr = rr; sp.delta = delta;
-            *spec_out = sp;
-            __hip_atomic_store(hres + 6, go ? 1.0 : 0.0, __ATOMIC_RELAXED, __HIP_MEMORY_SCOPE_SYSTEM);
-            __hip_atomic_store(hres + 7, delta, __ATOMIC_RELAXED, __HIP_MEMORY_SCOPE_SYSTEM);
-        }
-        __atomic_thread_fence(__ATOMIC_SEQ_CST);
-        asm volatile("s_waitcnt vmcnt(0)" ::: "memory");
-        __hip_atomic_store(reinterpret_cast<unsigned long long *>(hres + 5), seq, __ATOMIC_RELEASE, __HIP_MEMORY_SCOPE_SYSTEM);
-    }
+        publish_outer_result(hres, f, rr, m, sc, nullptr, seq);
+    }
+}
+
+template <int O>
+__global__ __launch_bounds__(256) void tcg_start_kernel(int nloc, const double *__restrict__ rgR, const double *__restrict__ rgs,
+                                                         const double *__restrict__ R, const double *__restrict__ s,
+                                                         double *rR, double *rs, double *pR, double *ps, double *vR, double *vs,
+                                                         double *HvR, double *Hvs, double *Wloc, TcgScal *scal0, unsigned long long *hstat,
+                                                         double *Wpad, int seq, const double *__restrict__ partsA, int nA_loc,
+                                                         const double *__restrict__ partsM, int nM, const TcgScal *scal_fin, double *hres,
+                                                         unsigned long long oseq, int grp, OuterArgs oa, unsigned int *arrive) {
+    __shared__ double sh[4];
+    __shared__ SpecCtl sh_sp;
+    __shared__ int sh_last;
+    double f = 0.0, rr = 0.0;
+    f += sum_partials256(partsA, nA_loc, sh, grp);
+    rr += sum_partials256(partsA + nA_loc, nA_loc, sh, grp);
+    const double m_vec = (nM > 0) ? sum_partials256(partsM, nM, sh, grp) : 0.0;
+    if (threadIdx.x == 0) {
+        const TcgScal sc = *scal_fin;
+        const double m = (nM > 0) ? m_vec : sc.model;
+        const SpecCtl sp = tr_decide(f, rr, m, sc, oa);
+        sh_sp = sp;
+        if (blockIdx.x == 0) publish_outer_result(hres, f, rr, m, sc, &sp, oseq);
+        __threadfence();
+        const unsigned int t = __hip_atomic_fetch_add(arrive, 1u, __ATOMIC_ACQ_REL, __HIP_MEMORY_SCOPE_AGENT);
+        sh_last = (t + 1 == gridDim.x);
+        if (sh_last) {
+            __hip_atomic_store(arrive, 0u, __ATOMIC_RELAXED, __HIP_MEMORY_SCOPE_AGENT);
+            TcgScal nx = {};
+            if (sp.go) {
+                nx.rr = sp.rr; nx.pp = sp.rr; nx.delta = sp.delta; nx.gradnorm = sqrt(sp.rr); nx.seq = seq;
+            } else {
+                nx = *scal0; nx.status = 9; nx.seq = seq;
+            }
+            *scal0 = nx;
+            if (sp.go) publish_host(hstat, pack_stat(seq, 0, 0));
+        }
+    }
+    __syncthreads();
+    if (!sh_sp.go) return;
+    tcg_init_vectors<O>(nloc, rgR, rgs, R, s, rR, rs, pR, ps, vR, vs, HvR, Hvs, Wloc, Wpad);
 }
 
 __device__ __forceinline__ double det3(const double (&M)[3][3]);
@@ -2264,7 +2309,7 @@
 }
 template <int O>
 static void qw_symv_epi(int epi, const double *Q, int64_t ld, const double *W, double alpha, const CamArgs &a, double *Prow, double *Pcol,
-                        hipStream_t st, int rev, unsigned long long *trace = nullptr) {
+                        hipStream_t st, int rev, unsigned long long *trace = nullptr, int part = 0) {
     const SymvPlan pl = symv_plan(a.nloc, ld);
     const int nstrips = (int)((ld + kSvStrip - 1) / kSvStrip);
     const TcgScal *sc = (epi == EPI_HESS || epi == EPI_AUTO) ? a.scal : (const TcgScal *)nullptr;
@@ -2272,9 +2317,11 @@
     const int ys = pl.ysplit, rK = 4 * pl.K, rKf = 4 * pl.Kf, rys = ys;
     const dim3 gs(pl.gx, pl.gy);
     const int nt0 = symv_nt_step0(a.nloc, ld);
-    if (trace) {
+    if (part == 2) {
+    } else if (trace) {
         if constexpr (O == 3 || O == 4) hipLaunchKernelGGL((qw_symv_kernel<O, true>), gs, dim3(256), 0, st, Q, ld, W, a.nloc, pl.K, pl.Kf, ys, nt0, sc, Prow, Pcol, trace, rev, by_phase);
     } else hipLaunchKernelGGL((qw_symv_kernel<O>), gs, dim3(256), 0, st, Q, ld, W, a.nloc, pl.K, pl.Kf, ys, nt0, sc, Prow, Pcol, trace, rev, by_phase);
+    if (part == 1) return;
     const dim3 g(qw_grid(a.nloc)), b(256);
     switch (epi) {
         case EPI_PLAIN: hipLaunchKernelGGL((symv_reduce_kernel<O, EPI_PLAIN>), g, b, 0, st, Prow, Pcol, ld, nstrips, rK, rKf, rys, alpha, a); break;
@@ -2302,13 +2349,13 @@
 }
 
 void launch_qw_sym(int o, int epi, const double *Q, int64_t ld, const double *W, double alpha, const CamArgs &a, double *Prow,
-                   double *Pcol, hipStream_t st, int rev) {
+                   double *Pcol, hipStream_t st, int rev, int part) {
     if (a.nloc <= 0) return;
     switch (o) {
-        case 1: qw_symv_epi<1>(epi, Q, ld, W, alpha, a, Prow, Pcol, st, rev & 1); break;
-        case 3: qw_symv_epi<3>(epi, Q, ld, W, alpha, a, Prow, Pcol, st, rev & 1); break;
-        case 4: qw_symv_epi<4>(epi, Q, ld, W, alpha, a, Prow, Pcol, st, rev & 1); break;
-        case 5: qw_symv_epi<5>(epi, Q, ld, W, alpha, a, Prow, Pcol, st, rev & 1); break;
+        case 1: qw_symv_epi<1>(epi, Q, ld, W, alpha, a, Prow, Pcol, st, rev & 1, nullptr, part); break;
+        case 3: qw_symv_epi<3>(epi, Q, ld, W, alpha, a, Prow, Pcol, st, rev & 1, nullptr, part); break;
+        case 4: qw_symv_epi<4>(epi, Q, ld, W, alpha, a, Prow, Pcol, st, rev & 1, nullptr, part); break;
+        case 5: qw_symv_epi<5>(epi, Q, ld, W, alpha, a, Prow, Pcol, st, rev & 1, nullptr, part); break;
         default: throw Error(-2, "symmetric product is instantiated for o = 1, 3..5");
     }
     check_launch("qw_symv");
@@ -2424,9 +2471,9 @@
 }
 void launch_tcg_init(int o, int nloc, const double *rgR, const double *rgs, const double *R, const double *s, double *rR, double *rs,
                      double *pR, double *ps, double *vR, double *vs, double *HvR, double *Hvs, double *Wloc, TcgScal *scal0,
-                     double rr, double delta, unsigned long long *hstat, hipStream_t st, double *Wpad, int seq, const SpecCtl *spec) {
+                     double rr, double delta, unsigned long long *hstat, hipStream_t st, double *Wpad, int seq) {
     XM_DISPATCH_O(o, hipLaunchKernelGGL((tcg_init_kernel<O_>), dim3(flat_grid((int64_t)nloc * 3 * pitch_of(O_))), dim3(256), 0, st,
-                                        nloc, rgR, rgs, R, s, rR, rs, pR, ps, vR, vs, HvR, Hvs, Wloc, scal0, rr, delta, hstat, Wpad, seq, spec));
+                                        nloc, rgR, rgs, R, s, rR, rs, pR, ps, vR, vs, HvR, Hvs, Wloc, scal0, rr, delta, hstat, Wpad, seq));
     check_launch("tcg_init");
 }
 void launch_cg_step(int o, int nloc, const TcgScal *scal_cur, TcgScal *scal_next, const double *parts, int nA_loc, int nB_loc, int world,
@@ -2440,12 +2487,17 @@
     check_launch("cg_step");
 }
 void launch_outer_finalize(const double *partsA, int nA_loc, int world, const double *partsM, int nM, const TcgScal *scal, double *hres,
-                           unsigned long long seq, int grouping, hipStream_t st, const OuterArgs *oa, SpecCtl *spec_out) {
-    OuterArgs z;
-    std::memset(&z, 0, sizeof(z));
-    hipLaunchKernelGGL(outer_finalize_kernel, dim3(1), dim3(256), 0, st, partsA, nA_loc, world, partsM, nM, scal, hres, seq, grouping, oa ? *oa : z,
-                       (oa != nullptr) ? spec_out : (SpecCtl *)nullptr);
+                           unsigned long long seq, int grouping, hipStream_t st) {
+    hipLaunchKernelGGL(outer_finalize_kernel, dim3(1), dim3(256), 0, st, partsA, nA_loc, world, partsM, nM, scal, hres, seq, grouping);
     check_launch("outer_finalize");
+}
+void launch_tcg_start(int o, int nloc, const double *rgR, const double *rgs, const double *R, const double *s, double *rR, double *rs,
+                      double *pR, double *ps, double *vR, double *vs, double *HvR, double *Hvs, double *Wloc, TcgScal *scal0,
+                      unsigned long long *hstat, hipStream_t st, double *Wpad, int seq, const OuterSums &os, const OuterArgs &oa, unsigned int *arrive) {
+    XM_DISPATCH_O(o, hipLaunchKernelGGL((tcg_start_kernel<O_>), dim3(flat_grid((int64_t)nloc * 3 * pitch_of(O_))), dim3(256), 0, st,
+                                        nloc, rgR, rgs, R, s, rR, rs, pR, ps, vR, vs, HvR, Hvs, Wloc, scal0, hstat, Wpad, seq, os.partsA, os.nA,
+                                        os.partsM, os.nM, os.scal_fin, os.hres, os.seq, os.grouping, oa, arrive));
+    check_launch("tcg_start");
 }
 void launch_outer_step(int o, int polar, const OuterStepArgs &A, int grid, hipStream_t st) {
     switch (o) {
@@ -2966,7 +3018,7 @@
 }
 template <int O>
 static void qw_symv_f32_epi(int epi, const float *Qf, const double *Qd, int64_t ld, const double *W, double alpha, const CamArgs &a, double *Prow,
-                            double *Pcol, hipStream_t st, int rev) {
+                            double *Pcol, hipStream_t st, int rev, int part) {
     const SymvPlan pl = symv_plan(a.nloc, ld);
     const int nstrips = (int)((ld + kSvStrip - 1) / kSvStrip);
     const int rK = 4 * pl.K, rKf = 4 * pl.Kf, ys = pl.ysplit;
@@ -2988,8 +3040,8 @@
             hipLaunchKernelGGL((symv_reduce_kernel<O, EPI_PLAIN>), g, b, 0, st, Prow, Pcol, ld, nstrips, rK, rKf, ys, alpha, a);
             break;
         case EPI_HESS:
-            hipLaunchKernelGGL((qw_symv_f32_kernel<O, false>), gs, b, 0, st, Qf, Qd, ld, W, a.nloc, pl.K, pl.Kf, ys, nt0, a.scal, Prow, Pcol, rev);
-            hipLaunchKernelGGL((symv_reduce_kernel<O, EPI_HESS>), g, b, 0, st, Prow, Pcol, ld, nstrips, rK, rKf, ys, alpha, a);
+            if (part != 2) hipLaunchKernelGGL((qw_symv_f32_kernel<O, false>), gs, b, 0, st, Qf, Qd, ld, W, a.nloc, pl.K, pl.Kf, ys, nt0, a.scal, Prow, Pcol, rev);
+            if (part != 1) hipLaunchKernelGGL((symv_reduce_kernel<O, EPI_HESS>), g, b, 0, st, Prow, Pcol, ld, nstrips, rK, rKf, ys, alpha, a);
             break;
         case EPI_AUTO:
             if constexpr (O >= 3) {
@@ -3004,12 +3056,13 @@
     }
 }
 void launch_qw_sym_f32(int o, int epi, const float *Qf, const double *Qd, int64_t ld, const double *W, double alpha, const CamArgs &a, double *Prow,
-                       double *Pcol, hipStream_t st, int rev) {
+                       double *Pcol, hipStream_t st, int rev, int part) {
     if (a.nloc <= 0) return;
+    if (part != 0 && epi != EPI_HESS) throw Error(-2, "fp32 symmetric product: only the Hessian pair is enqueued launch by launch");
     switch (o) {
-        case 3: qw_symv_f32_epi<3>(epi, Qf, Qd, ld, W, alpha, a, Prow, Pcol, st, rev & 1); break;
-        case 4: qw_symv_f32_epi<4>(epi, Qf, Qd, ld, W, alpha, a, Prow, Pcol, st, rev & 1); break;
-        case 5: qw_symv_f32_epi<5>(epi, Qf, Qd, ld, W, alpha, a, Prow, Pcol, st, rev & 1); break;
+        case 3: qw_symv_f32_epi<3>(epi, Qf, Qd, ld, W, alpha, a, Prow, Pcol, st, rev & 1, part); break;
+        case 4: qw_symv_f32_epi<4>(epi, Qf, Qd, ld, W, alpha, a, Prow, Pcol, st, rev & 1, part); break;
+        case 5: qw_symv_f32_epi<5>(epi, Qf, Qd, ld, W, alpha, a, Prow, Pcol, st, rev & 1, part); break;
         default: throw Error(-2, "fp32 symmetric product is instantiated for o = 3..5");
     }
     check_launch("qw_symv_f32");
diff --git a/xm-code_amd/csrc/xm_sell.h b/xm-code_amd/csrc/xm_sell.h
--- a/xm-code_amd/csrc/xm_sell.h
+++ b/xm-code_amd/csrc/xm_sell.h
@@ -87,7 +87,7 @@
 
 void check_viewgraph_blocks(const int64_t *rowptr, const int32_t *colidx, const double *blocks, int64_t nloc, int64_t row0);
 void launch_qw_sell(int o, int epi, SellMatrix &m, const double *W, double alpha, const CamArgs &a, int gm, hipStream_t st,
-                    const double *Wpad16 = nullptr);
+                    const double *Wpad16 = nullptr, int part = 0);
 bool sell_supports(int o);
 void sell_quat_roundtrip(const double block[9], double quat[4], double rebuilt[9]);
 
diff --git a/xm-code_amd/csrc/xm_sell.hip b/xm-code_amd/csrc/xm_sell.hip
--- a/xm-code_amd/csrc/xm_sell.hip
+++ b/xm-code_amd/csrc/xm_sell.hip
@@ -622,7 +622,7 @@
 }
 
 template <int O>
-static void qw_sell_o(int epi, SellMatrix &m, const double *W, double alpha, const CamArgs &a, int gm, hipStream_t st, const double *Wpad16) {
+static void qw_sell_o(int epi, SellMatrix &m, const double *W, double alpha, const CamArgs &a, int gm, hipStream_t st, const double *Wpad16, int part) {
     const TcgScal *sc = (epi == EPI_HESS) ? a.scal : (const TcgScal *)nullptr;
     double *parts = m.parts(O);
     SellArgs sa = m.args();
@@ -632,7 +632,7 @@
     const double *Wn = W;
     const int wn = sa.wstride;
     if (padded) { sa.wstride = 16; W = Wpad16; }
-    if (m.grid() > 0) {
+    if (m.grid() > 0 && part != 2) {
         const dim3 g(m.grid()), b(256);
         if (gm != 0 && (uint64_t)m.ncols() * (uint64_t)sa.wstride * 8u >= (1ull << 32)) gm = 0;
         sa.nt_off = m.nt_off(O, a.nloc);
@@ -650,6 +650,7 @@
             else hipLaunchKernelGGL((qw_sell_kernel<O, 0, PIPE>), g, b, 0, st, sa, W, sc, parts);
         }
     }
+    if (part == 1) return;
     const dim3 g(m.reduce_grid(O, a.nloc)), b(256);
 #define XM_SELL_REDUCE(GW_)                                                                                                                          \
     switch (epi) {                                                                                                                                  \
@@ -662,9 +663,10 @@
 #undef XM_SELL_REDUCE
 }
 
-void launch_qw_sell(int o, int epi, SellMatrix &m, const double *W, double alpha, const CamArgs &a, int gm, hipStream_t st, const double *Wpad16) {
+void launch_qw_sell(int o, int epi, SellMatrix &m, const double *W, double alpha, const CamArgs &a, int gm, hipStream_t st, const double *Wpad16, int part) {
     if (a.nloc <= 0) return;
     if (epi == EPI_CERT) {
+        if (part != 0) throw Error(XM_ERR_ARG, "certificate operator: both launches at once");
         if (o != 1) throw Error(XM_ERR_ARG, "certificate operator needs o == 1");
         double *parts = m.parts(1);
         SellArgs sa = m.args();
@@ -678,10 +680,10 @@
         else hipLaunchKernelGGL((sell_reduce_kernel<1, EPI_CERT, 16>), dim3(m.reduce_grid(1, a.nloc)), dim3(256), 0, st, sa.pptr, sa.ridx, parts, alpha, a, sa.diag, W, sa.row0, sa.wstride);
     } else {
         switch (o) {
-            case 1: qw_sell_o<1>(epi, m, W, alpha, a, 0, st, nullptr); break;
-            case 3: qw_sell_o<3>(epi, m, W, alpha, a, gm, st, Wpad16); break;
-            case 4: qw_sell_o<4>(epi, m, W, alpha, a, gm, st, Wpad16); break;
-            case 5: qw_sell_o<5>(epi, m, W, alpha, a, gm, st, Wpad16); break;
+            case 1: qw_sell_o<1>(epi, m, W, alpha, a, 0, st, nullptr, part); break;
+            case 3: qw_sell_o<3>(epi, m, W, alpha, a, gm, st, Wpad16, part); break;
+            case 4: qw_sell_o<4>(epi, m, W, alpha, a, gm, st, Wpad16, part); break;
+            case 5: qw_sell_o<5>(epi, m, W, alpha, a, gm, st, Wpad16, part); break;
             default: throw Error(XM_ERR_ARG, "SELL product is instantiated for o = 1, 3, 4, 5");
         }
     }
diff --git a/xm-code_amd/csrc/xm_solver.h b/xm-code_amd/csrc/xm_solver.h
--- a/xm-code_amd/csrc/xm_solver.h
+++ b/xm-code_amd/csrc/xm_solver.h
@@ -252,6 +252,7 @@
     bool verbose_ = false;
     std::vector<std::pair<hipEvent_t, hipEvent_t>> ev_pool_;
     size_t ev_used_ = 0;
+    bool ev_open_ = false;
     int64_t hess_launches_ = 0;
     int sym_rev_ = 1;
     std::vector<float> qw_samples_;
@@ -270,17 +271,20 @@
     CamArgs cam_args(int state) const;
     int prod_grid() const;
     int tcg_blocks() const;
-    void product(int epi, int o, double alpha, const CamArgs &a);
+    void product(int epi, int o, double alpha, const CamArgs &a, int part = 0);
     void gather_W();
     void flush_gather();
     bool overlap_applies() const;
     void eval_point(int state, const double *Rp, const double *sp, double &f, double &rr);
     double sum_parts(const double *dparts, int count);
     int run_tcg(double rr, double delta, TcgScal &fin, int adopted = 0);
-    int enqueue_spec_tcg();
-    void tcg_enqueue_iteration(int i, bool profile);
+    void enqueue_spec_tcg(const OuterSums &os, const OuterArgs &oa);
+    void tcg_enqueue_iteration(int i, bool profile, int part = 0);
+    void tcg_enqueue_unit(bool profile);
+    int tcg_it_ = 0;
+    bool tcg_half_ = false;
+    DevBuf<unsigned int> spec_arrive_;
     bool spec_applies() const;
-    DevBuf<SpecCtl> spec_;
     unsigned int tcg_seq_ = 0;
     volatile double *wait_outer_result();
     bool stream_idle(std::chrono::steady_clock::time_point t_wait, const char *what);
diff --git a/xm-code_amd/csrc/xm_solver.hip b/xm-code_amd/csrc/xm_solver.hip
--- a/xm-code_amd/csrc/xm_solver.hip
+++ b/xm-code_amd/csrc/xm_solver.hip
@@ -485,7 +485,7 @@
         Pstrip_.alloc(mat);
     }
     scal_.ensure(2, st_);
-    spec_.ensure(1, st_);
+    spec_arrive_.ensure(1, st_);
     if (sell_ && sell_supports(o)) (void)sell_->parts(o);
     ensure_pinned(std::max<size_t>((size_t)2 * nA_ + (size_t)nB_ + partsM_.count + 64, (size_t)ld_ * OP_ + (size_t)ntot_ + 1024));
     if (comm_->active()) comm_->host_barrier();
@@ -557,7 +557,7 @@
     return a;
 }
 
-void Context::product(int epi, int o, double alpha, const CamArgs &a) {
+void Context::product(int epi, int o, double alpha, const CamArgs &a, int part) {
     if (w_pending_) {
         if (storage_ == XM_STORAGE_DENSE && (epi == EPI_PLAIN || epi == EPI_GRAD) && o == o_) {
             w_pending_ = false;
@@ -580,22 +580,22 @@
         flush_gather();
     }
     if (storage_ == XM_STORAGE_DENSE && dQ32_ && o == o_ && (epi == EPI_HESS || epi == EPI_AUTO)) {
-        if (sym_ok_ && o >= 3 && o <= sym_max_o_ && Pcol_.p) launch_qw_sym_f32(o, epi, dQ32_, dQ_, ld_, W_.p, alpha, a, Prow_.p, Pcol_.p, st_, sym_rev_);
-        else { CamArgs ar = a; ar.rev = sym_rev_; launch_qw_dense_f32(o, epi, dQ32_, dQ_, ld_, W_.p, alpha, ar, st_); }
+        if (sym_ok_ && o >= 3 && o <= sym_max_o_ && Pcol_.p) launch_qw_sym_f32(o, epi, dQ32_, dQ_, ld_, W_.p, alpha, a, Prow_.p, Pcol_.p, st_, sym_rev_, part);
+        else if (part != 2) { CamArgs ar = a; ar.rev = sym_rev_; launch_qw_dense_f32(o, epi, dQ32_, dQ_, ld_, W_.p, alpha, ar, st_); }
     } else if (storage_ == XM_STORAGE_DENSE) {
-        if (symw_ && o == o_ && o >= 3 && o <= sym_max_o_ && epi != EPI_CERT) product_symw(epi, o, alpha, a);
-        else if (sym_ok_ && o == o_ && o >= 3 && o <= sym_max_o_ && epi != EPI_CERT && Pcol_.p) launch_qw_sym(o, epi, dQ_, ld_, W_.p, alpha, a, Prow_.p, Pcol_.p, st_, sym_rev_);
-        else { CamArgs ar = a; ar.rev = sym_rev_; launch_qw_dense(o, epi, dQ_, ld_, W_.p, alpha, ar, st_); }
+        if (symw_ && o == o_ && o >= 3 && o <= sym_max_o_ && epi != EPI_CERT) { if (part != 2) product_symw(epi, o, alpha, a); }
+        else if (sym_ok_ && o == o_ && o >= 3 && o <= sym_max_o_ && epi != EPI_CERT && Pcol_.p) launch_qw_sym(o, epi, dQ_, ld_, W_.p, alpha, a, Prow_.p, Pcol_.p, st_, sym_rev_, part);
+        else if (part != 2) { CamArgs ar = a; ar.rev = sym_rev_; launch_qw_dense(o, epi, dQ_, ld_, W_.p, alpha, ar, st_); }
     } else if (storage_ == XM_STORAGE_SCHUR) {
-        schur_->product(o, epi, W_.p, alpha, a, st_);
+        if (part != 2) schur_->product(o, epi, W_.p, alpha, a, st_);
     } else if (sell_ && sell_supports(o)) {
         const double *wp = (epi == EPI_HESS && o == o_) ? wpad() : ((epi == EPI_GRAD && o == o_) ? wpad_next_ : nullptr);
         wpad_next_ = nullptr;
-        launch_qw_sell(o, epi, *sell_, W_.p, alpha, a, sell_gm_, st_, wp);
-    } else {
+        launch_qw_sell(o, epi, *sell_, W_.p, alpha, a, sell_gm_, st_, wp, part);
+    } else if (part != 2) {
         launch_qw_bsr3(o, epi, rowptr_.p, colidx_.p, blocks_.p, W_.p, alpha, a, st_, nb_loc_, rowinfo_.p);
     }
-    if (res_) res_->qw_products++;
+    if (res_ && part != 2) res_->qw_products++;
 }
 
 int Context::product_kind(int o) const {
@@ -706,6 +706,7 @@
         float ms = 0.f;
         if (hipEventElapsedTime(&ms, ev_pool_[i].first, ev_pool_[i].second) == hipSuccess) qw_samples_.push_back(ms);
     }
+    if (ev_open_ && ev_used_ > 0) std::swap(ev_pool_[0], ev_pool_[ev_used_]);
     ev_used_ = 0;
 }
 
@@ -720,7 +721,7 @@
     qw_samples_.clear();
 }
 
-void Context::tcg_enqueue_iteration(int i, bool profile) {
+void Context::tcg_enqueue_iteration(int i, bool profile, int part) {
     const int nA_loc = prod_grid(), nB_loc = tcg_blocks();
     const int rank = comm_->rank;
     const bool fused = xchg_.world > 1;
@@ -738,14 +739,17 @@
     double *pcur = pB + (size_t)par * chunk * comm_->world, *pnext = pB + (size_t)(par ^ 1) * chunk * comm_->world;
     a.partials = pcur + (size_t)rank * chunk + b_off;
     a.Bout = comm_->active() ? pcur + (size_t)rank * chunk : nullptr;
-    const bool timed = profile && (hess_launches_ % kProfileStride == 0) && ev_used_ < ev_pool_.size();
-    if (timed) XM_HIP_CHECK(hipEventRecord(ev_pool_[ev_used_].first, st_));
+    if (part != 2) {
+        ev_open_ = profile && (hess_launches_ % kProfileStride == 0) && ev_used_ < ev_pool_.size();
+        if (ev_open_) XM_HIP_CHECK(hipEventRecord(ev_pool_[ev_used_].first, st_));
+        hess_launches_++;
+    }
     const bool model_rec = opt_ && (opt_->flags & XM_FLAG_MODEL_RECURRENCE);
     sym_rev_ = par;
-    product(EPI_HESS, o_, 2.0, a);
+    product(EPI_HESS, o_, 2.0, a, part);
     sym_rev_ = 1;
-    if (timed) { XM_HIP_CHECK(hipEventRecord(ev_pool_[ev_used_].second, st_)); ev_used_++; }
-    hess_launches_++;
+    if (part == 1) return;
+    if (ev_open_) { XM_HIP_CHECK(hipEventRecord(ev_pool_[ev_used_].second, st_)); ev_used_++; ev_open_ = false; }
     if (lockstep) comm_->allgather(pcur, chunk, st_);
     launch_cg_step(o_, nloc_, scal_.p + par, scal_.p + (par ^ 1), pcur, nA_loc, nB_loc, comm_->world, HpR_.p, Hps_.p, R_.p,
                    s_.p, pR_.p, par ? psB_.p : psA_.p, par ? psA_.p : psB_.p, vR_.p, vs_.p, model_rec ? nullptr : HvR_.p, model_rec ? nullptr : Hvs_.p, rR_.p,
@@ -757,21 +761,27 @@
     return !comm_->active() && opt_ && !(opt_->flags & XM_FLAG_HOST_STEPPED) && storage_ != XM_STORAGE_SCHUR && cfg_.debug_drop_finalize < 0;
 }
 
-int Context::enqueue_spec_tcg() {
+void Context::enqueue_spec_tcg(const OuterSums &os, const OuterArgs &oa) {
     std::swap(R_.p, Rc_.p);
     std::swap(s_.p, sc_.p);
     cur_ ^= 1;
     const PointState &P = ps_[cur_];
     double *Wloc = wpad() ? nullptr : W_.p + (size_t)cam0_ * 3 * OP_;
     ++tcg_seq_;
-    launch_tcg_init(o_, nloc_, P.rgR.p, P.rgs.p, R_.p, s_.p, rR_.p, rs_.p, pR_.p, psA_.p, vR_.p, vs_.p, HvR_.p, Hvs_.p, Wloc,
-                    scal_.p, 0.0, 0.0, hstat_dev_, st_, wpad(), (int)tcg_seq_, spec_.p);
-    const int n_spec = 1;
-    for (int i = 0; i < n_spec; ++i) tcg_enqueue_iteration(i, false);
+    launch_tcg_start(o_, nloc_, P.rgR.p, P.rgs.p, R_.p, s_.p, rR_.p, rs_.p, pR_.p, psA_.p, vR_.p, vs_.p, HvR_.p, Hvs_.p, Wloc, scal_.p, hstat_dev_, st_,
+                     wpad(), (int)tcg_seq_, os, oa, spec_arrive_.p);
+    tcg_it_ = 0;
+    tcg_enqueue_iteration(0, false, 1);
+    tcg_half_ = true;
     std::swap(R_.p, Rc_.p);
     std::swap(s_.p, sc_.p);
     cur_ ^= 1;
-    return n_spec;
+}
+
+void Context::tcg_enqueue_unit(bool profile) {
+    tcg_enqueue_iteration(tcg_it_++, profile, 2);
+    tcg_half_ = false;
+    if (tcg_it_ < kMaxInner) { tcg_enqueue_iteration(tcg_it_, profile, 1); tcg_half_ = true; }
 }
 
 int Context::run_tcg(double rr, double delta, TcgScal &fin, int adopted) {
@@ -791,7 +801,10 @@
     const bool lockstep = comm_->active() && !fused;
     const int run_ahead = (lockstep || prod_grid() >= 64) ? 2 : 3;
     int fin_status = 0, fin_iter = 0;
-    int it = adopted;
+    const bool by_launch = spec_applies() && !stepped;
+    const int depth = (prod_grid() >= 64) ? 1 : 3;
+    if (by_launch && adopted == 0) { tcg_it_ = 0; tcg_enqueue_iteration(0, profile, 1); tcg_half_ = true; }
+    int it = by_launch ? tcg_it_ : adopted;
     auto enqueue = [&](int i) { tcg_enqueue_iteration(i, profile); };
     auto read_scal = [&](int par) {
         TcgScal sc;
@@ -816,6 +829,9 @@
             const int status = valid ? (int)(v & 0xff) : 0;
             const int done = valid ? (int)((v >> 8) & 0xffffff) : 0;
             if (status != 0) { fin_status = status; fin_iter = done; break; }
+            if (by_launch) {
+                if (tcg_half_ && tcg_it_ - done < depth) { tcg_enqueue_unit(profile); it = tcg_it_; continue; }
+            } else
             if (it < kMaxInner && it - done < run_ahead) { enqueue(it++); continue; }
             __builtin_ia32_pause();
             if (secs_since(last_progress) > 200e-6) {
@@ -824,7 +840,7 @@
                     if (sc.status != 0) { fin_status = sc.status; fin_iter = sc.iter; break; }
                     if (it >= kMaxInner) { fin_status = 6; fin_iter = kMaxInner; break; }
                     *hstat_ = ((unsigned long long)tcg_seq_ << 32) | ((unsigned long long)(unsigned)sc.iter << 8);
-                    if (it - sc.iter >= run_ahead) enqueue(it++);
+                    if (!by_launch && it - sc.iter >= run_ahead) enqueue(it++);
                 }
                 last_progress = clk::now();
             }
@@ -943,12 +959,14 @@
         }
         const long long drop_at = cfg_.debug_drop_finalize;
         const bool spec = spec_applies();
-        const OuterArgs oa = {loss, delta, delta_bar, gradtol, shrink_count, (k + 1 >= kMaxOuter) ? 1 : 0};
-        if (drop_at >= 0 && (long long)outer_seq_ + 1 == drop_at) ++outer_seq_;
-        else
-        launch_outer_finalize(partsA_.p, nA_loc, comm_->world, partsM_.p, model_rec ? 0 : nB_loc * comm_->world, scal_.p + (enq & 1),
-                              reinterpret_cast<double *>(hstat_dev_) + 8, ++outer_seq_, grouping_, st_, spec ? &oa : nullptr, spec_.p);
-        const int n_spec = spec ? enqueue_spec_tcg() : 0;
+        double *hres_dev = reinterpret_cast<double *>(hstat_dev_) + 8;
+        const int nM = model_rec ? 0 : nB_loc * comm_->world;
+        if (spec) {
+            const OuterArgs oa = {loss, delta, delta_bar, gradtol, shrink_count, (k + 1 >= kMaxOuter) ? 1 : 0};
+            const OuterSums os = {partsA_.p, nA_loc, partsM_.p, nM, scal_.p + (enq & 1), hres_dev, ++outer_seq_, grouping_};
+            enqueue_spec_tcg(os, oa);
+        } else if (drop_at >= 0 && (long long)outer_seq_ + 1 == drop_at) ++outer_seq_;
+        else launch_outer_finalize(partsA_.p, nA_loc, comm_->world, partsM_.p, nM, scal_.p + (enq & 1), hres_dev, ++outer_seq_, grouping_, st_);
         volatile double *hres = wait_outer_result();
         double f_new = hres[0], rr_new = hres[1], loss_qu = hres[2];
         const bool spec_go = spec && hres[6] != 0.0;
@@ -960,7 +978,6 @@
         endreason = fin.status;
         inner_print = fin.iter + 1;
         totalite += fin.iter + 1;
-        if (opt_->flags & XM_FLAG_PROFILE_QW) drain_events();
         if (loss_qu >= 0) { log("error! loss_qu is larger than 0\n"); stop_reason = 12; break; }
         const double rou = (f_new - loss) / loss_qu;
         if (rou < 0.25) { delta *= 0.25; trstatus = 1; shrink_count++; }
@@ -980,11 +997,12 @@
             if (stop_delta) { stop_reason = 13; break; }
             loss = f_new;
             rr = rr_new;
-            if (spec_go && std::memcmp(&spec_delta, &delta, sizeof(double)) == 0) adopted = n_spec;
+            if (spec_go && std::memcmp(&spec_delta, &delta, sizeof(double)) == 0) { adopted = 1; tcg_enqueue_unit((opt_->flags & XM_FLAG_PROFILE_QW) != 0); }
         } else {
             trstatus = 3;
         }
-        if (n_spec > 0 && adopted != n_spec && res_) res_->qw_products -= n_spec;
+        if (spec && !adopted && res_) res_->qw_products -= 1;
+        if (opt_->flags & XM_FLAG_PROFILE_QW) drain_events();
     }
     log("\nTotal iteration:     %lld\n", totalite);
     const double secs = secs_since(start);
@@ -1906,6 +1924,7 @@
         for (auto &e : ev_pool_) { XM_HIP_CHECK(hipEventCreate(&e.first)); XM_HIP_CHECK(hipEventCreate(&e.second)); }
     }
     ev_used_ = 0;
+    ev_open_ = false;
     hess_launches_ = 0;
     qw_samples_.clear();
     const auto t0 = clk::now();
```

Measured after the change: 24500, median of 4. About the same (+0.2%).
